# JJanai/slowflow

Hardware: AMD Instinct MI355X
Metric: Mpix*solver-iters/s at 1024x436 (whole coarse-to-fine path) (higher is better)
Workload: dtype f32

## Files before the change

slowflow_amd/csrc/api.hip:

```cpp
#include <algorithm>
#include <cmath>
#include <cstring>
#include <memory>
#include <mutex>

#include "sfa_internal.h"

#pragma clang fp contract(off)

namespace sfa {

thread_local std::string g_thread_err;

#ifndef SFA_RELEASE
Switches g_switches;
static const char *const kSwitchNames[Switches::N] = {
    "SFA_SOR_CHAIN", "SFA_SOR_BAND", "SFA_SOR_F", "SFA_SOR_CH", "SFA_SOR_LEAD", "SFA_CHAIN_LDS", "SFA_RB_TILE", "SFA_WARP_ALLJ", "SFA_NO_WARP_SMOOTH",
    "SFA_ASSEMBLE_GENERIC", "SFA_EXACT_DIV", "SFA_ASM_XCD", "SFA_NO_DIRECT_OPERANDS", "SFA_NO_UV_ALIAS", "SFA_DEBUG_ACTIVE", "SFA_UNFUSED", "SFA_SHARE_SOR",
    "SFA_PYRAMID_UNFUSED", "SFA_CUT_DISCHARGE", "SFA_CUT_INNER", "SFA_CUT_SUPER", "SFA_CUT_TAIL_INNER", "SFA_CUT_PER", "SFA_CUT_TAIL_PER", "SFA_CUT_TAIL_SUPER",
    "SFA_CUT_DEBUG", "SFA_CUT_NO_TAIL", "SFA_CUT_TAIL", "SFA_NO_EXACT_BREAK", "SFA_PAIR_UNFUSED"};
static int set_switch(const char *name, const char *value) {
    for (int i = 0; i < Switches::N; i++)
        if (!strcmp(name, kSwitchNames[i])) {
            g_switches.given[i] = value != nullptr;
            g_switches.value[i] = value ? atoi(value) : 0;
            return SFA_OK;
        }
    return SFA_ERR_ARG;
}
static void switches_from_environment() {
    static std::once_flag once;
    std::call_once(once, [] {
        const char *d = getenv("SFA_DEBUG");
        if (!d || atoi(d) == 0) return;
        for (int i = 0; i < Switches::N; i++)
            if (const char *e = getenv(kSwitchNames[i])) (void)set_switch(kSwitchNames[i], e);
    });
}
#else
static void switches_from_environment() {}
#endif

int set_error(sfa_ctx *ctx, int code, const char *fmt, ...) {
    char buf[1024];
    va_list ap;
    va_start(ap, fmt);
    vsnprintf(buf, sizeof buf, fmt, ap);
    va_end(ap);
    g_thread_err = buf;
    if (ctx) ctx->err = buf;
    return code;
}

int DevMem::alloc(sfa_ctx *ctx, size_t n) {
    if (n <= bytes && p) return SFA_OK;
    release();
    hipError_t e = hipMalloc(&p, n);
    if (e != hipSuccess) { p = nullptr; return set_error(ctx, SFA_ERR_HIP, "hipMalloc(%zu) failed: %s", n, hipGetErrorString(e)); }
    bytes = n;
    return SFA_OK;
}
void DevMem::release() {
    if (p) (void)hipFree(p);
    p = nullptr;
    bytes = 0;
}

int upload_plane(sfa_ctx *ctx, float *dev, int pitch, const float *host, int stride, int w, int h) {
    SFA_HIP(ctx, hipMemcpy2DAsync(dev, (size_t)pitch * 4, host, (size_t)stride * 4, (size_t)w * 4, h, hipMemcpyHostToDevice, ctx->stream));
    return SFA_OK;
}
int download_plane(sfa_ctx *ctx, float *host, int stride, const float *dev, int pitch, int w, int h) {
    SFA_HIP(ctx, hipMemcpy2DAsync(host, (size_t)stride * 4, dev, (size_t)pitch * 4, (size_t)w * 4, h, hipMemcpyDeviceToHost, ctx->stream));
    return SFA_OK;
}

static int check_device_error(sfa_ctx *c) {
    unsigned e = 0;
    SFA_HIP(c, hipMemcpyAsync(&e, c->d_err, sizeof e, hipMemcpyDeviceToHost, c->stream));
    SFA_HIP(c, hipStreamSynchronize(c->stream));
    if (e) {
        (void)hipMemsetAsync(c->d_err, 0, sizeof(unsigned), c->stream);
        return set_error(c, SFA_ERR_TIMEOUT, "SOR pipeline: a bounded in-kernel wait gave up (code %u)", e);
    }
    return SFA_OK;
}

int cv_gauss_taps(float sigma, float *k) {
    const int ksize = ((int)lrint((double)sigma * 4 * 2 + 1)) | 1;
    const double scale2X = -0.5 / ((double)sigma * sigma);
    double sum = 0;
    for (int i = 0; i < ksize; i++) {
        const double x = i - (ksize - 1) * 0.5;
        k[i] = (float)exp(scale2X * x * x);
        sum += k[i];
    }
    sum = 1. / sum;
    for (int i = 0; i < ksize; i++) k[i] = (float)(k[i] * sum);
    return ksize / 2;
}

}

using namespace sfa;

extern "C" {

int sfa_device_count(void) {
    int n = 0;
    if (hipGetDeviceCount(&n) != hipSuccess) return 0;
    return n;
}

int sfa_ctx_create(int device, sfa_ctx **out) {
    if (!out) return set_error(nullptr, SFA_ERR_ARG, "sfa_ctx_create: out is null");
    *out = nullptr;
    int n = 0;
    if (hipGetDeviceCount(&n) != hipSuccess || n <= 0)
        return set_error(nullptr, SFA_ERR_NO_DEVICE, "no HIP device available: slowflow_amd has no CPU fallback");
    if (device < 0 || device >= n) return set_error(nullptr, SFA_ERR_ARG, "device %d out of range (%d devices)", device, n);
    switches_from_environment();
    std::unique_ptr<sfa_ctx> c(new sfa_ctx());
    c->device = device;
    SFA_HIP(c.get(), hipSetDevice(device));
    SFA_HIP(c.get(), hipStreamCreateWithFlags(&c->stream, hipStreamNonBlocking));
    SFA_HIP(c.get(), hipMalloc((void **)&c->d_red, kRedDoubles * sizeof(double)));
    SFA_HIP(c.get(), hipHostMalloc((void **)&c->h_red, sizeof(LastBlock) + 64, hipHostMallocDefault));
    SFA_HIP(c.get(), hipMalloc((void **)&c->d_amask, 64));
    SFA_HIP(c.get(), hipMalloc((void **)&c->d_last, sizeof(LastBlock)));
    SFA_HIP(c.get(), hipMemset(c->d_last, 0, sizeof(LastBlock)));
    SFA_HIP(c.get(), hipHostMalloc((void **)&c->h_amask, kMaskRing * sizeof(WMask), hipHostMallocDefault));
    for (auto &e : c->ev_mask) SFA_HIP(c.get(), hipEventCreateWithFlags(&e, hipEventDisableTiming));
    SFA_HIP(c.get(), hipMalloc((void **)&c->d_err, 64));
    SFA_HIP(c.get(), hipMemset(c->d_err, 0, 64));
    SFA_HIP(c.get(), hipEventCreate(&c->t0));
    SFA_HIP(c.get(), hipEventCreate(&c->t1));
    SFA_HIP(c.get(), hipEventCreateWithFlags(&c->ev_wait, hipEventDisableTiming));
    SFA_HIP(c.get(), hipEventCreateWithFlags(&c->ev_signal, hipEventDisableTiming));
    hipDeviceProp_t prop;
    if (hipGetDeviceProperties(&prop, device) == hipSuccess) c->cu_count = prop.multiProcessorCount;
    *out = c.release();
    return SFA_OK;
}

void sfa_ctx_destroy(sfa_ctx *c) {
    if (!c) return;
    (void)hipSetDevice(c->device);
    (void)hipStreamSynchronize(c->stream);
    for (auto e : c->ev) (void)hipEventDestroy(e);
    for (auto e : c->ev2) (void)hipEventDestroy(e);
    if (c->t0) (void)hipEventDestroy(c->t0);
    if (c->t1) (void)hipEventDestroy(c->t1);
    if (c->ev_wait) (void)hipEventDestroy(c->ev_wait);
    if (c->ev_signal) (void)hipEventDestroy(c->ev_signal);
    if (c->d_red) (void)hipFree(c->d_red);
    if (c->h_red) (void)hipHostFree(c->h_red);
    if (c->d_err) (void)hipFree(c->d_err);
    if (c->d_amask) (void)hipFree(c->d_amask);
    if (c->d_last) (void)hipFree(c->d_last);
    if (c->h_amask) (void)hipHostFree(c->h_amask);
    for (auto e : c->ev_mask) if (e) (void)hipEventDestroy(e);
    if (c->rb_tmp) (void)hipFree(c->rb_tmp);
    if (c->q_tmp) (void)hipFree(c->q_tmp);
    if (c->stream) (void)hipStreamDestroy(c->stream);
    delete c;
}

const char *sfa_last_error(const sfa_ctx *c) { return c ? c->err.c_str() : g_thread_err.c_str(); }

int sfa_ctx_sync(sfa_ctx *c) {
    if (!c) return set_error(nullptr, SFA_ERR_ARG, "null context");
    SFA_HIP(c, hipSetDevice(c->device));
    return check_device_error(c);
// ... 774 lines not shown
```

slowflow_amd/csrc/job.hip:

```cpp
#include <algorithm>
#include <cmath>
#include <cstring>
#include <memory>
#include <vector>

#include "sfa_internal.h"

#pragma clang fp contract(off)

namespace sfa {

enum { P_WX = 0, P_WY, P_UU, P_VV, P_DU, P_DV, P_ODU, P_ODV, P_SH, P_SV, P_A11, P_A12, P_A22, P_B1, P_B2, P_OCC, P_DPSIS, P_COUNT };
struct Level {
    int w = 0, h = 0, pitch = 0, lstride = 0, ref = 0, F = 0, nb = 0;
    bool fused = true;
    long pl = 0, es = 0;
    long off_masks = 0, off_warp = 0, off_stacks = 0, off_tmp = 0;
    float *base = nullptr;
    float *pbase = nullptr;
    float *plane(int i) const { return i < 2 ? pbase + (long)i * pl : base + (long)(i - 2) * pl; }
    float *mask(int s) const { return base + off_masks + (long)s * pl; }
    float *stack(int s, int toref) const { return base + off_stacks + ((long)s * 2 + toref) * 24 * pl; }
    float *warp(int s, int sp1) const { return base + off_warp + (long)(s + sp1) * 3 * pl; }
    float *frame(int f) const { return pbase + 2 * pl + (long)f * 3 * pl; }
    float *tmp() const { return base + off_tmp; }
    Geo geo() const { return Geo{w, h, pitch, pl, es, nb, WMask::first(nb), nullptr}; }
    Geo geo(const WMask &active) const { return Geo{w, h, pitch, pl, es, nb, active, nullptr}; }
    static long persistent_floats(int pitch, int h, int ref) { return (long)pitch * h * (2 + (2L * ref + 1) * 3); }
    static long transient_floats(int pitch, int h, int ref, bool fused) {
        return (long)pitch * h * ((P_COUNT - 2) + 2 * ref + (2L * ref + 1) * 3 + (fused ? 0 : 2L * ref * 2 * 24));
    }
    void layout(float *transient, float *persistent, int w_, int h_, int lstride_, int ref_, int nb_, long es_, bool fused_) {
        base = transient; pbase = persistent; w = w_; h = h_; pitch = dev_pitch(w_); lstride = lstride_; ref = ref_; F = 2 * ref_ + 1; nb = nb_; es = es_; fused = fused_;
        pl = (long)pitch * h;
        off_masks = (long)(P_COUNT - 2) * pl;
        off_warp = off_masks + 2L * ref * pl;
        off_stacks = off_warp + (2L * ref + 1) * 3 * pl;
        off_tmp = off_warp;
    }
};
struct ChannelWeights { const float *dev = nullptr; long pl = 0, es = 0; int pitch = 0, stride0 = 0; };

static const float *pair_image(const Level &L, int s, int sp1) { return (s + sp1 - L.ref == 0) ? L.frame(s + sp1) : L.warp(s, sp1); }

static bool get_derivatives(sfa_ctx *c, const Level &L, const sfa_params &p, const Geo &g, const bool need_toref[2 * SFA_MAX_REF], bool with_smoothness = false) {
    const int ref = L.ref;
    WarpJobs J;
    J.n = 0;
    for (int f = p.one_direction ? ref + 1 : 0; f <= 2 * ref; f++) {
        if (f == ref) continue;
        const int s = f < ref ? f : f - 1;
        J.job[J.n++] = WarpJob{L.frame(f) - L.base, L.warp(f < ref ? f : f - 1, f < ref ? 0 : 1) - L.base, L.mask(s) - L.base, f - ref};
    }
    const bool smoothed = with_smoothness && L.fused &&
                          launch_warp_smooth(c, g, J, L.base, L.plane(P_WX), L.plane(P_WY), p.smoothing, L.plane(P_SH), L.plane(P_SV), L.plane(P_DPSIS), p.alpha, pen(p.robust_reg));
    if (!smoothed) launch_warp_jobs(c, g, J, L.base, L.plane(P_WX), L.plane(P_WY));
    for (int s = p.one_direction ? ref : 0; s < 2 * ref; s++) {
        if (L.fused) continue;
        const float *w_s = pair_image(L, s, 0), *w_sp1 = pair_image(L, s, 1);
        launch_deriv_stack(c, g, L.stack(s, 0), w_s, w_sp1, L.es, L.es);
        if (need_toref[s]) {
            if (s < ref) launch_deriv_stack(c, g, L.stack(s, 1), w_s, L.frame(ref), L.es, L.es);
            else         launch_deriv_stack(c, g, L.stack(s, 1), L.frame(ref), w_sp1, L.es, L.es);
        }
    }
    return smoothed;
}

static int optimize_occlusions(sfa_ctx *c, const Level &L, const sfa_params &p, const Geo &g, DevMem &scratch) {
    const int ref = L.ref;
    const size_t n = (size_t)L.nb * L.pl;
    SFA_TRY(scratch.alloc(c, (2 + kCutWorkPlanes) * n * sizeof(float)));
    float *d0 = scratch.f(), *d1 = d0 + n, *work = d1 + n;
    OccArgs oa;
    memset(&oa, 0, sizeof oa);
    oa.nslots = 2 * ref; oa.hd = p.delta / 3.0f; oa.hg = p.gamma / 3.0f; oa.penalty = p.occlusion_penalty;
    oa.color = pen(p.robust_color); oa.grad = pen(p.robust_grad);
    for (int s = 0; s < 2 * ref; s++) {
        const float *i1 = pair_image(L, s, 0), *i2 = pair_image(L, s, 1);
        const float *r1 = s < ref ? i1 : L.frame(ref), *r2 = s < ref ? L.frame(ref) : i2;
        const int idx = std::max(ref - s - 1, s - ref);
        oa.slot[s] = OccSlot{i1 - L.base, i2 - L.base, r1 - L.base, r2 - L.base, L.off_masks + (long)s * L.pl, p.rho[idx], p.omega[idx], s >= ref ? 0 : 1};
    }
    launch_occ_costs(c, g, oa, L.base, d0, d1, L.pl);
    return run_grid_cut(c, g, L.plane(P_OCC), L.es, d0, d1, work, p.occlusion_alpha);
}


static Term data_term(const Level &L, const sfa_params &p, int slot, int is_ref, float weight, float s) {
    const float *i1 = pair_image(L, slot, 0), *i2 = pair_image(L, slot, 1);
    if (is_ref) { if (slot < L.ref) i2 = L.frame(L.ref); else i1 = L.frame(L.ref); }
    return Term{L.off_stacks + ((long)slot * 2 + is_ref) * 24 * L.pl, L.off_masks + (long)slot * L.pl, weight * (p.delta / 3.0f), weight * (p.gamma / 3.0f), s, is_ref,
                i1 - L.base, i2 - L.base, slot < L.ref};
}
static int data_terms(sfa_ctx *c, const Level &L, const sfa_params &p, const ChannelWeights &cw, AssembleArgs &aa, bool need_toref[2 * SFA_MAX_REF]) {
    const int ref = L.ref;
    memset(&aa, 0, sizeof aa);
    for (int s = 0; s < ref; s++) {
        const int a = ref - 1 - s;
        if (!p.one_direction) {
            if (p.rho[a] > 0) aa.t[aa.n++] = data_term(L, p, s, 0, p.rho[a], (float)(s - ref));
            if (p.omega[a] > 0) { aa.t[aa.n++] = data_term(L, p, s, 1, p.omega[a], (float)(s - ref)); need_toref[s] = true; }
        }
        if (p.rho[s] > 0) aa.t[aa.n++] = data_term(L, p, ref + s, 0, p.rho[s], (float)s);
        if (p.omega[s] > 0) { aa.t[aa.n++] = data_term(L, p, ref + s, 1, p.omega[s], (float)(s + 1)); need_toref[ref + s] = true; }
        aa.data_norm += p.rho[s] + p.omega[s];
    }
    for (int t = 0; t < aa.n; t++)
        if (aa.t[t].is_ref && aa.t[t].s == 0) return set_error(c, SFA_ERR_REF_FRAME, "Frame compared to reference frame is the reference frame itself!");
    aa.one_direction = p.one_direction; aa.dt_norm = p.dataterm_norm;
    aa.color = pen(p.robust_color); aa.grad = pen(p.robust_grad);
    aa.chw = cw.dev; aa.chw_pl = cw.pl; aa.chw_es = cw.es; aa.chw_pitch = cw.pitch; aa.chw_stride0 = cw.stride0; aa.lstride = L.lstride;
    aa.accumulate = 0; aa.do_laplacian = 1;
    return SFA_OK;
}

struct LevelPlan {
    bool verbose;
    bool red_black;
    bool direct;
    bool uv_alias;
    bool thres_in, thres_out;
    float *wx, *wy, *uu, *vv, *du, *dv, *odu, *odv, *sh, *sv, *a11, *a12, *a22, *b1, *b2, *occ, *dpsis, *UU, *VV;
    float *dfa, *dfb, *ifa, *ifb;
    LevelPlan(const sfa_ctx *c, const Level &L, const sfa_params &p) {
        verbose = c->verbose_changes;
        red_black = p.sor_order == 1;
        direct = L.fused && !red_black && !sw_given(Switches::NO_DIRECT_OPERANDS);
        uv_alias = direct && p.niter_inner == 1 && !sw_given(Switches::NO_UV_ALIAS) && !verbose;
        thres_in = p.thres_inner > 0; thres_out = p.thres_outer > 0;
        wx = L.plane(P_WX); wy = L.plane(P_WY); uu = L.plane(P_UU); vv = L.plane(P_VV); du = L.plane(P_DU); dv = L.plane(P_DV);
        odu = L.plane(P_ODU); odv = L.plane(P_ODV); sh = L.plane(P_SH); sv = L.plane(P_SV); a11 = L.plane(P_A11); a12 = L.plane(P_A12);
        a22 = L.plane(P_A22); b1 = L.plane(P_B1); b2 = L.plane(P_B2); occ = L.plane(P_OCC); dpsis = L.plane(P_DPSIS);
        UU = uv_alias ? wx : uu; VV = uv_alias ? wy : vv;
        dfa = thres_out && !sw_given(Switches::NO_EXACT_BREAK) ? a11 : nullptr; dfb = dfa ? a12 : nullptr;
        ifa = thres_in && !sw_given(Switches::NO_EXACT_BREAK) ? a11 : nullptr; ifb = ifa ? a12 : nullptr;
    }
};

struct OuterBreak {
    sfa_ctx *c; bool on;
    int known(int n, WMask &active) const {
        if (!on || n < kMaskLag) return SFA_OK;
        const int slot = (n - kMaskLag) % kMaskRing;
        SFA_HIP(c, hipEventSynchronize(c->ev_mask[slot]));
        for (int i = 0; i < kMaskWords; i++) active.w[i] = *(volatile unsigned long long *)&c->h_amask[slot].w[i];
        return SFA_OK;
    }
    int publish(int n) const {
        if (!on) return SFA_OK;
        const int slot = n % kMaskRing;
        SFA_HIP(c, hipMemcpyAsync(&c->h_amask[slot], c->d_amask, sizeof(WMask), hipMemcpyDeviceToHost, c->stream));
        SFA_HIP(c, hipEventRecord(c->ev_mask[slot], c->stream));
        return SFA_OK;
    }
};

static void print_changes(sfa_ctx *c, const Level &L, const char *what, int it, const WMask &who) {
    if (hipMemcpyAsync(c->h_red, c->d_red, 2 * L.nb * sizeof(double), hipMemcpyDeviceToHost, c->stream) != hipSuccess || hipStreamSynchronize(c->stream) != hipSuccess) return;
    const double n = (double)L.w * L.h;
    for (int b = 0; b < L.nb; b++)
        if (who.test(b)) {
            if (L.nb > 1) printf("[window %d] ", b);
            printf("%s %d\tavg change %g,%g\n", what, it, (double)(float)(c->h_red[2 * b] / n), (double)(float)(c->h_red[2 * b + 1] / n));
        }
    fflush(stdout);
}

static int assemble_and_solve(sfa_ctx *c, const Level &L, const sfa_params &p, const LevelPlan &P, AssembleArgs &aa, SorWorkspace &sorws, const Geo &gi, bool first_zero,
                       bool smoothed) {
    if (!first_zero) launch_copy_planes(c, gi, P.odu, P.du, 2, L.es, L.es);
    if (!smoothed) launch_smoothness(c, gi, p.smoothing, P.sh, P.sv, P.UU, P.VV, P.dpsis, p.alpha, pen(p.robust_reg));
    aa.op = SorOperandOut();
    aa.zero_duv = first_zero ? 1 : 0;
    if (P.direct) SFA_TRY(sor_operand_target(c, sorws, gi, p.niter_solver, &aa.op));
    if (L.fused) SFA_TRY(launch_assemble_images(c, gi, aa, L.base, P.a11, P.a12, P.a22, P.b1, P.b2, P.du, P.dv, P.UU, P.VV, P.sh, P.sv, P.occ));
    else launch_assemble(c, gi, aa, L.base, P.a11, P.a12, P.a22, P.b1, P.b2, P.du, P.dv, P.uu, P.vv, P.sh, P.sv);
    if (P.direct) return sor_run_prepared(c, sorws, gi, nullptr, nullptr, p.niter_solver, p.sor_omega);
    if (P.red_black) return sor_rb_run(c, gi, P.du, P.dv, P.a11, P.a12, P.a22, P.b1, P.b2, P.sh, P.sv, p.niter_solver, p.sor_omega);
    return sor_run(c, sorws, gi, P.du, P.dv, P.a11, P.a12, P.a22, P.b1, P.b2, P.sh, P.sv, p.niter_solver, p.sor_omega, false);
}

static bool update_flow(sfa_ctx *c, const sfa_params &p, const LevelPlan &P, const SorOperandOut &x, const Geo &gi, int inner, bool first_zero) {
    const bool last = inner + 1 == p.niter_inner;
    float *const ia = last ? nullptr : P.ifa, *const ib = last ? nullptr : P.ifb;
    if (P.direct && last && !P.verbose) {
        launch_update_outer_x(c, gi, P.uv_alias ? nullptr : P.uu, P.uv_alias ? nullptr : P.vv, P.wx, P.wy, x, c->d_red, P.dfa, P.dfb);
        return true;
    }
    if (P.direct)
        launch_update_inner_x(c, gi, P.uu, P.vv, P.wx, P.wy, x, first_zero ? nullptr : P.odu, first_zero ? nullptr : P.odv, last ? nullptr : P.du,
                              last ? nullptr : P.dv, c->d_red, ia, ib);
    else
        launch_update_inner(c, gi, P.uu, P.vv, P.wx, P.wy, P.du, P.dv, P.odu, P.odv, c->d_red, ia, ib);
    return false;
}

static int inner_break(sfa_ctx *c, const Level &L, const sfa_params &p, const LevelPlan &P, const Geo &gi, WMask &in_active) {
    const double npx = (double)L.h * L.w;
    SFA_HIP(c, hipMemcpyAsync(c->h_red, c->d_red, 2 * L.nb * sizeof(double), hipMemcpyDeviceToHost, c->stream));
    SFA_HIP(c, hipStreamSynchronize(c->stream));
    WMask close = WMask::none();
    for (int b = 0; b < L.nb; b++)
        if (in_active.test(b)) {
            const double ad = c->h_red[2 * b] / npx, dd = c->h_red[2 * b + 1] / npx, dm = (ad < dd) ? dd : ad;
            if (P.ifa && fabs(dm - (double)p.thres_inner) <= break_band(L.w, L.h) * (double)p.thres_inner) { close.set(b); continue; }
            if (std::max((float)ad, (float)dd) < p.thres_inner) in_active.clear(b);
        }
    if (!close.any()) return SFA_OK;
    float *const dx = c->d_last->exact;
    const float *const hx = reinterpret_cast<const LastBlock *>(c->h_red)->exact;
    launch_exact_norms(c, gi, P.ifa, P.ifb, close, dx);
    SFA_HIP(c, hipMemcpyAsync(const_cast<float *>(hx), dx, 2 * L.nb * sizeof(float), hipMemcpyDeviceToHost, c->stream));
    SFA_HIP(c, hipStreamSynchronize(c->stream));
    for (int b = 0; b < L.nb; b++)
        if (close.test(b) && std::max(hx[2 * b], hx[2 * b + 1]) < p.thres_inner) in_active.clear(b);
    return SFA_OK;
}

static int inner_iterations(sfa_ctx *c, const Level &L, const sfa_params &p, const LevelPlan &P, AssembleArgs &aa, SorWorkspace &sorws, const Geo &g, bool smoothed) {
    if (!P.direct) launch_zero_planes(c, g, P.du, 2);
    WMask in_active = g.active, outer_done = WMask::none();
    for (int inner = 0; inner < p.niter_inner; inner++) {
        Geo gi = g;
        gi.active = in_active;
        const bool first_zero = P.direct && inner == 0;
        SFA_TRY(assemble_and_solve(c, L, p, P, aa, sorws, gi, first_zero, smoothed && inner == 0));
        if (update_flow(c, p, P, aa.op, gi, inner, first_zero)) outer_done = in_active;
        if (P.verbose) print_changes(c, L, "\tinner it", inner, in_active);
        if (P.thres_in && inner + 1 < p.niter_inner) {
            SFA_TRY(inner_break(c, L, p, P, gi, in_active));
            if (!in_active.any()) break;
        }
    }
    if (outer_done != g.active) {
        Geo go = g;
        go.active = g.active.andnot(outer_done);
        launch_update_outer(c, go, P.wx, P.wy, P.uu, P.vv, c->d_red, P.dfa, P.dfb);
    }
    return SFA_OK;
}
static int run_level(sfa_ctx *c, const Level &L, const sfa_params &p, const ChannelWeights &cw, SorWorkspace &sorws, DevMem &cut_scratch, float *change, float *occ_log) {
    AssembleArgs aa;
    bool need_toref[2 * SFA_MAX_REF] = {false};
    SFA_TRY(data_terms(c, L, p, cw, aa, need_toref));
    const LevelPlan P(c, L, p);
    const OuterBreak brk{c, P.thres_out};
    const WMask all = WMask::first(L.nb);
    Geo g = L.geo(all);
    launch_fill_planes(c, g, P.occ, 1, (p.one_direction || p.occlusion_reasoning) ? -1.0f : 0.0f);
    launch_dpsis(c, g, P.dpsis, L.frame(L.ref), L.es, 5.0f, p.norm_avg, p.norm_std, p.hbit);
    if (!P.uv_alias) launch_copy_planes(c, g, P.uu, P.wx, 2, L.es, L.es);
    g.amask = c->d_amask;
    SFA_HIP(c, hipMemsetAsync(c->d_last, 0, sizeof(LastBlock), c->stream));
    launch_set_mask(c, all);

    for (int alter = 0; alter < p.niter_alter; alter++) {
        WMask active = all;
        g.active = active;
        if (P.thres_out && alter > 0) launch_set_mask(c, all);
        bool smoothed = get_derivatives(c, L, p, g, need_toref, P.uv_alias);
        if (alter > 0 && p.occlusion_reasoning && !p.one_direction) SFA_TRY(optimize_occlusions(c, L, p, g, cut_scratch));
        if (alter > 0 && p.occlusion_reasoning && occ_log)
            launch_copy_planes(c, g, occ_log + (long)alter * L.pl, P.occ, 1, (long)p.niter_alter * L.pl, L.es);
        for (int outer = 0; outer < p.niter_outer; outer++) {
            SFA_TRY(brk.known(outer, active));
            if (!active.any()) break;
            if (sw_given(Switches::DEBUG_ACTIVE)) fprintf(stderr, "level %dx%d alter %d outer %d known active %d\n", L.w, L.h, alter, outer, active.count());
            g.active = active;
            if (outer > 0) smoothed = get_derivatives(c, L, p, g, need_toref, P.uv_alias);
            if (!L.fused) launch_mask_weight(c, g, L.mask(0), P.occ, aa.data_norm, L.ref, p.one_direction);
            SFA_TRY(inner_iterations(c, L, p, P, aa, sorws, g, smoothed));
            if (P.verbose) print_changes(c, L, "outer it", outer, active);
            const bool last_iter = (alter == p.niter_alter - 1 && outer == p.niter_outer - 1);
            if (P.thres_out || last_iter) launch_outer_threshold(c, g, c->d_red, P.thres_out ? p.thres_outer : 0.0f, P.dfa, P.dfb);
            SFA_TRY(brk.publish(outer));
        }
    }
    if (change) {
        SFA_HIP(c, hipMemcpyAsync(c->h_red, c->d_last->last, 2 * L.nb * sizeof(double), hipMemcpyDeviceToHost, c->stream));
        SFA_HIP(c, hipStreamSynchronize(c->stream));
        for (int i = 0; i < 2 * L.nb; i++) change[i] = (float)c->h_red[i];
    }
    return SFA_OK;
}

static int gaussian_filter_order(float sigma) {
    int order = (int)floor(3 * sigma) + 1;
    if (order == 0) order = 1;
    return order;
}
static int pyramid_sizes(int w, int h, int layers, float p_scale, int *ws, int *hs) {
    const float sigma = 1 / sqrtf(2 * p_scale);
    const int order = gaussian_filter_order(sigma);
    for (int l = 0; l < layers; l++) {
        ws[l] = l == 0 ? w : (int)(float)floor(ws[l - 1] * p_scale);
        hs[l] = l == 0 ? h : (int)(float)floor(hs[l - 1] * p_scale);
        if (floor(ws[l] * p_scale) <= order + 1 || floor(hs[l] * p_scale) <= order + 1) return l;
    }
    return layers;
}

}
using namespace sfa;

struct sfa_job {
    sfa_ctx *ctx = nullptr;
    sfa_params p;
    int w = 0, h = 0, nb = 0, ref = 0, F = 0, L = 0;
    int ws[64], hs[64];
    long es = 0;
    std::vector<long> level_off;
    long trans_off = 0;
    bool share_sor = false;
    DevMem arena;
    DevMem init_flow;
    DevMem chw;
    DevMem cut_scratch;
    bool has_chw = false;
    int chw_stride0 = 0;
    std::vector<std::unique_ptr<SorWorkspace>> sor;
    std::vector<float> change;
    double mpix_iters = 0;
    int host_stride0 = 0;
    bool fused = true;
    Level level(int l) const {
        Level Lv;
        Lv.layout(arena.f() + trans_off, arena.f() + level_off[l], ws[l], hs[l], l == 0 ? host_stride0 : host_stride(ws[l]), ref, nb, es, fused);
        return Lv;
    }
    WMask presmoothed = WMask::none();
    bool keep_alt_occ = false;
    DevMem occ_log;
    float *chw_stage = nullptr;
    hipEvent_t ev_chw = nullptr;
};

static int job_windows(sfa_ctx *ctx, const char *fn, const sfa_job *j, int b0, int n) { return check_batch_range(ctx, fn, "windows", b0, n, j->nb); }

static int job_weight_planes(sfa_job *j, int stride) {
    if (j->has_chw) return SFA_OK;
    const size_t n = (size_t)j->nb * 3 * dev_pitch(stride) * j->h;
    SFA_TRY(j->chw.alloc(j->ctx, n * sizeof(float)));
    launch_fill(j->ctx, j->chw.f(), n, 1.0f);
    j->has_chw = true;
    j->chw_stride0 = stride;
    return SFA_OK;
}
static int job_set_channel_weights(sfa_job *j, int b, int stride, const float *const chw[3]) {
    sfa_ctx *ctx = j->ctx;
    if (chw) {
        CHECK_ARGS((long)stride * j->h < (1L << 31), "channel weights: the linear pixel index must fit 31 bits");
        SFA_TRY(job_weight_planes(j, stride));
        CHECK_ARGS(j->chw_stride0 == stride, "channel weights of all elements must share one stride");
        const int cp = dev_pitch(stride);
        for (int k = 0; k < 3; k++) {
            CHECK_ARGS(chw[k], "null weight plane");
            SFA_TRY(upload_plane(ctx, j->chw.f() + ((long)b * 3 + k) * cp * j->h, cp, chw[k], stride, stride, j->h));
        }
    } else if (j->has_chw) {
        launch_fill(ctx, j->chw.f() + (long)b * 3 * dev_pitch(j->chw_stride0) * j->h, (size_t)3 * dev_pitch(j->chw_stride0) * j->h, 1.0f);
    }
    return SFA_OK;
}
static int job_upload_flow_and_weights(sfa_job *j, int b, const float *wx, const float *wy, int stride, const float *const chw[3]) {
    sfa_ctx *ctx = j->ctx;
    const Level L0 = j->level(0);
    const float *const host[2] = {wx, wy};
    for (int k = 0; k < 2; k++) {
        float *dst = j->init_flow.f() + ((long)b * 2 + k) * L0.pl;
        if (host[k]) SFA_TRY(upload_plane(ctx, dst, L0.pitch, host[k], stride, j->w, j->h));
        else SFA_HIP(ctx, hipMemsetAsync(dst, 0, L0.pl * sizeof(float), ctx->stream));
    }
    return job_set_channel_weights(j, b, stride, chw);
}
static void job_presmooth(sfa_job *j) {
    const WMask all = WMask::first(j->nb);
    if (!(j->p.presmooth_sigma > 0) || (j->presmoothed & all) == all) return;
    const Level L0 = j->level(0);
    float *tmp = L0.tmp();
    for (int f = 0; f < j->F; f++) {
        launch_presmooth(j->ctx, L0.geo(all), tmp + 3 * L0.pl, tmp, L0.frame(f), 3, j->p.presmooth_sigma);
        launch_copy_planes(j->ctx, L0.geo(all.andnot(j->presmoothed)), L0.frame(f), tmp + 3 * L0.pl, 3, L0.es, L0.es);
    }
    j->presmoothed = all;
}
static void job_pyramid(sfa_job *j) {
    sfa_ctx *ctx = j->ctx;
    const int nb = j->nb, F = j->F;
    float taps[64];
    const int radius = cv_gauss_taps(1 / sqrtf(2 * j->p.p_scale), taps);
    for (int l = 1; l < j->L; l++) {
        const Level Lp = j->level(l - 1), Lc = j->level(l);
        float *tmp = Lp.tmp();
        if (!sw_given(Switches::PYRAMID_UNFUSED) &&
            launch_pyr_down(ctx, Lc.frame(0), Lc.w, Lc.h, Lc.pitch, Lc.pl, Lc.es, Lp.frame(0), Lp.w, Lp.h, Lp.pitch, Lp.pl, Lp.es, 3 * F, nb, taps, radius))
            continue;
        for (int f = 0; f < F; f++) {
            launch_gauss_blur(ctx, Lp.geo(), tmp + 3 * Lp.pl, tmp, Lp.frame(f), 3, taps, radius);
            launch_resize(ctx, Lc.frame(f), Lc.w, Lc.h, Lc.pitch, Lc.pl, Lc.es, tmp + 3 * Lp.pl, Lp.w, Lp.h, Lp.pitch, Lp.pl, Lp.es, 3, nb, 1.0f);
        }
    }
}
static void job_initial_flow(sfa_job *j) {
    const Level L0 = j->level(0), Lt = j->level(j->L - 1);
    if (j->L > 1) {
        const float fx = (1.0f * Lt.w) / j->w, fy = (1.0f * Lt.h) / j->h;
        launch_resize_flow(j->ctx, Lt.plane(P_WX), Lt.plane(P_WY), Lt.w, Lt.h, Lt.pitch, Lt.es, j->init_flow.f(), j->init_flow.f() + L0.pl, j->w, j->h, L0.pitch, 2 * L0.pl, j->nb, fx, fy);
    } else {
        launch_copy_planes(j->ctx, L0.geo(), L0.plane(P_WX), j->init_flow.f(), 2, L0.es, 2 * L0.pl);
    }
}

extern "C" {

int sfa_pyramid_sizes(int w, int h, int layers, float p_scale, int *ws, int *hs) {
    if (layers < 1 || layers > 64 || !ws || !hs) return 0;
    return pyramid_sizes(w, h, layers, p_scale, ws, hs);
}

int sfa_job_create(sfa_ctx *ctx, const sfa_params *p, int w, int h, int batch, sfa_job **out) {
    CHECK_ARGS(ctx && p && out && w >= 2 && h >= 5 && batch > 0 && batch <= kMaxBatch, "bad arguments (h >= 5, w >= 2)");
    CHECK_ARGS(p->S >= 2 && p->S - 1 <= SFA_MAX_REF && p->layers >= 1 && p->layers <= 64, "unsupported slow_flow_S / slow_flow_layers");
    CHECK_ARGS(2L * kMaxBatch + 2L * batch * ((w + 63) / 64) * 16 <= kRedDoubles, "batch x width beyond the change norms' scratch (sfa_internal.h: kRedDoubles)");
    SFA_HIP(ctx, hipSetDevice(ctx->device));
    std::unique_ptr<sfa_job> j(new sfa_job());
    j->ctx = ctx; j->p = *p; j->w = w; j->h = h; j->nb = batch; j->ref = p->S - 1; j->F = 2 * j->ref + 1;
    j->L = pyramid_sizes(w, h, p->layers, p->p_scale, j->ws, j->hs);
    CHECK_ARGS(j->L >= 1, "image too small for even one pyramid level");
    j->fused = sw_int(Switches::UNFUSED, 0) == 0;
    long off = 0;
    double px = 0;
    for (int l = 0; l < j->L; l++) {
        j->level_off.push_back(off);
        off += Level::persistent_floats(dev_pitch(j->ws[l]), j->hs[l], j->ref);
        j->sor.emplace_back(new SorWorkspace());
        px += (double)j->ws[l] * j->hs[l];
    }
    j->trans_off = off;
    off += Level::transient_floats(dev_pitch(j->ws[0]), j->hs[0], j->ref, j->fused);
    j->es = off;
    j->share_sor = (double)w * h >= 2.0e6 || sw_given(Switches::SHARE_SOR);
    j->host_stride0 = host_stride(w);
    SFA_TRY(j->arena.alloc(ctx, (size_t)batch * j->es * sizeof(float)));
    SFA_HIP(ctx, hipMemsetAsync(j->arena.p, 0, (size_t)batch * j->es * sizeof(float), ctx->stream));
    SFA_TRY(j->init_flow.alloc(ctx, (size_t)batch * 2 * dev_pitch(w) * h * sizeof(float)));
    SFA_HIP(ctx, hipMemsetAsync(j->init_flow.p, 0, (size_t)batch * 2 * dev_pitch(w) * h * sizeof(float), ctx->stream));
    j->change.assign(2 * batch, 0.f);
    j->mpix_iters = px * p->niter_alter * p->niter_outer * p->niter_inner * p->niter_solver * batch / 1e6;
    *out = j.release();
    return SFA_OK;
}
void sfa_job_destroy(sfa_job *j) {
    if (!j) return;
    (void)hipSetDevice(j->ctx->device);
    (void)hipStreamSynchronize(j->ctx->stream);
    if (j->ev_chw) (void)hipEventDestroy(j->ev_chw);
    if (j->chw_stage) (void)hipHostFree(j->chw_stage);
    delete j;
}
double sfa_job_mpix_iters(const sfa_job *j) { return j ? j->mpix_iters : 0; }
double sfa_job_device_bytes(const sfa_job *j) {
    if (!j) return 0;
    double b = (double)j->arena.bytes + j->init_flow.bytes + j->chw.bytes + j->cut_scratch.bytes + j->occ_log.bytes;
    for (const auto &w : j->sor) b += (double)w->sa.bytes + w->sb.bytes + w->x.bytes + w->flags.bytes + w->order.bytes + w->edge.bytes;
    return b;
}

int sfa_job_upload(sfa_job *j, int b, const float *const *frames, int n_frames, const float *wx, const float *wy, int stride, const float *const chw[3]) {
    sfa_ctx *ctx = j ? j->ctx : nullptr;
    CHECK_ARGS(j && b >= 0 && b < j->nb && frames && n_frames == j->F && stride >= j->w, "bad arguments (n_frames must be 2*(S-1)+1)");
    SFA_HIP(ctx, hipSetDevice(ctx->device));
    Level L0 = j->level(0);
    j->host_stride0 = stride;
    j->presmoothed.clear(b);
    for (int f = 0; f < j->F; f++) {
        CHECK_ARGS(frames[f], "null frame");
        for (int k = 0; k < 3; k++)
            SFA_TRY(upload_plane(ctx, L0.frame(f) + b * j->es + k * L0.pl, L0.pitch, frames[f] + (size_t)k * stride * j->h, stride, j->w, j->h));
    }
    SFA_TRY(job_upload_flow_and_weights(j, b, wx, wy, stride, chw));
    SFA_HIP(ctx, hipStreamSynchronize(ctx->stream));
    return SFA_OK;
}

int sfa_job_upload_resident(sfa_job *j, int b, const sfa_sequence *q, const int *frame_index, int n_frames, const float *wx, const float *wy, int stride,
                            const float *const chw[3]) {
    sfa_ctx *ctx = j ? j->ctx : nullptr;
    CHECK_ARGS(j && q && frame_index && b >= 0 && b < j->nb && n_frames == j->F && stride >= j->w, "bad arguments (n_frames must be 2*(S-1)+1)");
    CHECK_ARGS(q->w == j->w && q->h == j->h && q->ctx->device == ctx->device, "the sequence must have the job's frame size and live on the job's GPU");
    SFA_HIP(ctx, hipSetDevice(ctx->device));
    Level L0 = j->level(0);
    j->host_stride0 = stride;
    j->presmoothed.clear(b);
    for (int f = 0; f < j->F; f++) {
        CHECK_ARGS(frame_index[f] >= 0 && frame_index[f] < q->n, "frame index out of range");
        SFA_HIP(ctx, hipMemcpyAsync(L0.frame(f) + b * j->es, q->frame(frame_index[f]), (size_t)3 * L0.pl * sizeof(float), hipMemcpyDeviceToDevice, ctx->stream));
    }
    SFA_TRY(job_upload_flow_and_weights(j, b, wx, wy, stride, chw));
    if (wx || wy || chw) SFA_HIP(ctx, hipStreamSynchronize(ctx->stream));
    return SFA_OK;
}

int sfa_job_reset_flow(sfa_job *j) { return j ? SFA_OK : SFA_ERR_ARG; }

int sfa_job_run(sfa_job *j) {
    sfa_ctx *ctx = j ? j->ctx : nullptr;
    CHECK_ARGS(j, "null job");
    SFA_HIP(ctx, hipSetDevice(ctx->device));
    job_presmooth(j);
    job_pyramid(j);
    job_initial_flow(j);
    ChannelWeights cw;
    if (j->has_chw) {
        cw.dev = j->chw.f(); cw.pitch = dev_pitch(j->chw_stride0); cw.pl = (long)cw.pitch * j->h; cw.es = 3 * cw.pl; cw.stride0 = j->chw_stride0;
    }
    for (int l = j->L - 1; l >= 0; l--) {
        Level Lc = j->level(l);
        if (l < j->L - 1) {
            Level Ln = j->level(l + 1);
            const float fx = (1.0f * Lc.w) / Ln.w, fy = (1.0f * Lc.h) / Ln.h;
            launch_resize_flow(ctx, Lc.plane(P_WX), Lc.plane(P_WY), Lc.w, Lc.h, Lc.pitch, Lc.es, Ln.plane(P_WX), Ln.plane(P_WY), Ln.w, Ln.h, Ln.pitch, Ln.es, j->nb, fx, fy);
        }
        SFA_TRY(run_level(ctx, Lc, j->p, cw, *j->sor[j->share_sor ? 0 : l], j->cut_scratch, l == 0 ? j->change.data() : nullptr, l == 0 && j->keep_alt_occ ? j->occ_log.f() : nullptr));
    }
    SFA_HIP(ctx, hipGetLastError());
    return SFA_OK;
}

int sfa_job_download(sfa_job *j, int b, float *wx, float *wy, int stride, float change[2]) {
    sfa_ctx *ctx = j ? j->ctx : nullptr;
    CHECK_ARGS(j && b >= 0 && b < j->nb && wx && wy && stride >= j->w, "bad arguments");
    SFA_HIP(ctx, hipSetDevice(ctx->device));
    Level L0 = j->level(0);
    SFA_TRY(download_plane(ctx, wx, stride, L0.plane(P_WX) + b * j->es, L0.pitch, j->w, j->h));
    SFA_TRY(download_plane(ctx, wy, stride, L0.plane(P_WY) + b * j->es, L0.pitch, j->w, j->h));
    if (change) { change[0] = j->change[2 * b]; change[1] = j->change[2 * b + 1]; }
    return sfa_ctx_sync(ctx);
}

int sfa_job_keep_alternation_occlusions(sfa_job *j, int on) {
    sfa_ctx *ctx = j ? j->ctx : nullptr;
    CHECK_ARGS(j, "null job");
    SFA_HIP(ctx, hipSetDevice(ctx->device));
    j->keep_alt_occ = on != 0;
    if (on) {
        const size_t n = (size_t)j->nb * std::max(1, j->p.niter_alter) * dev_pitch(j->w) * j->h * sizeof(float);
        SFA_TRY(j->occ_log.alloc(ctx, n));
        SFA_HIP(ctx, hipMemsetAsync(j->occ_log.p, 0, n, ctx->stream));
    }
    return SFA_OK;
}

int sfa_job_download_alternation_occlusions(sfa_job *j, int b, int alter, float *occ, int stride) {
    sfa_ctx *ctx = j ? j->ctx : nullptr;
    CHECK_ARGS(j && b >= 0 && b < j->nb && occ && stride >= j->w, "bad arguments");
    CHECK_ARGS(j->keep_alt_occ && j->occ_log.p, "sfa_job_keep_alternation_occlusions was not enabled before the run");
    CHECK_ARGS(alter >= 1 && alter < j->p.niter_alter, "alternation out of range: labels exist for 1 <= alter < niter_alter (variational_mt.cpp:269)");
    SFA_HIP(ctx, hipSetDevice(ctx->device));
    const int pitch = dev_pitch(j->w);
    const long pl = (long)pitch * j->h;
    SFA_TRY(download_plane(ctx, occ, stride, j->occ_log.f() + ((long)b * j->p.niter_alter + alter) * pl, pitch, j->w, j->h));
    return sfa_ctx_sync(ctx);
}

int sfa_job_download_occlusions(sfa_job *j, int b, float *occ, int stride) {
    sfa_ctx *ctx = j ? j->ctx : nullptr;
    CHECK_ARGS(j && b >= 0 && b < j->nb && occ && stride >= j->w, "bad arguments");
    SFA_HIP(ctx, hipSetDevice(ctx->device));
    Level L0 = j->level(0);
    SFA_TRY(download_plane(ctx, occ, stride, L0.plane(P_OCC) + b * j->es, L0.pitch, j->w, j->h));
    return sfa_ctx_sync(ctx);
}

int sfa_job_upload_device(sfa_job *j, int b0, int n, const void *frames_dev, const sfa_dev_layout *l, const float *const chw[3]) {
    sfa_ctx *ctx = j ? j->ctx : nullptr;
    CHECK_ARGS(j, "job is null");
    SFA_HIP(ctx, hipSetDevice(ctx->device));
    SFA_TRY(job_windows(ctx, __func__, j, b0, n));
    SFA_TRY(check_frames_source(ctx, __func__, frames_dev, l, l ? l->window : 0, n, j->F, j->w, j->h));
    const int stride = host_stride(j->w);
    if (chw) {
        CHECK_ARGS(chw[0] && chw[1] && chw[2], "chw holds a null weight plane");
        CHECK_ARGS(!j->has_chw || j->chw_stride0 == stride, "chw: the job already holds channel weights of another stride");
    }
    Level L0 = j->level(0);
    j->host_stride0 = stride;
    for (int b = b0; b < b0 + n; b++) j->presmoothed.clear(b);
    const PackSrc src{frames_dev, l->dtype, l->window, l->frame, l->channel, l->row, l->column};
    launch_pack_frames(ctx, L0.frame(0) + (long)b0 * j->es, j->es, L0.pl, L0.pitch, j->w, j->h, n, j->F, src);
    if (chw) {
        const size_t plane = (size_t)stride * j->h;
        if (!j->chw_stage) {
            SFA_HIP(ctx, hipHostMalloc((void **)&j->chw_stage, 3 * plane * sizeof(float), hipHostMallocDefault));
            SFA_HIP(ctx, hipEventCreateWithFlags(&j->ev_chw, hipEventDisableTiming));
        } else {
            SFA_HIP(ctx, hipEventSynchronize(j->ev_chw));
        }
// ... 88 lines not shown
```

slowflow_amd/csrc/kernels.hip:

```cpp
#include "sfa_device.h"
#include "sor_device.h"

#pragma clang fp contract(off)

namespace sfa {

__device__ __forceinline__ float psi_vec(const PenaltyDev &p, float xsq) {
    const float e2 = p.eps * p.eps;
    switch (p.id) {
    case 0: return 1.0f;
    case 2: return __fdiv_rn(1.0f, 2.0f * e2 + xsq);
    case 3: {
        float out = __fdiv_rn(1.0f, 2.0f * sqrt_rn(xsq + e2));
        if (sqrt_rn(xsq) > p.trunc) out = 0.0f;
        return out;
    }
    case 4: {
        float t = e2 + xsq;
        t = t * t;
        return __fdiv_rn(e2 + 2.0f * xsq, t);
    }
    default: return __fdiv_rn(1.0f, 2.0f * sqrt_rn(xsq + e2));
    }
}
// ... 547 lines not shown
        tmp = uxsq + vxsq;
        outh = (float)((double)((dps(x, y) + dps(x + 1, y)) * half_alpha) / __dsqrt_rn((double)(tmp + EPS2F)));
    }
    if (y < h - 1) {
        const float uy1 = uu(x, y + 1) - uu(x, y), vy1 = vv(x, y + 1) - vv(x, y);
        float tmp = 0.5f * (d3x(uu, x, y, w) + d3x(uu, x, y + 1, w));
        const float uysq = uy1 * uy1 + tmp * tmp;
        tmp = 0.5f * (d3x(vv, x, y, w) + d3x(vv, x, y + 1, w));
        const float vysq = vy1 * vy1 + tmp * tmp;
        tmp = uysq + vysq;
        outv = (float)((double)((dps(x, y) + dps(x, y + 1)) * half_alpha) / __dsqrt_rn((double)(tmp + EPS2F)));
    }
    sh[o] = outh;
    sv[o] = outv;
}
void launch_smoothness_2f(sfa_ctx *c, const Geo &g, float *sh, float *sv, const float *uu, const float *vv, const float *dpsis, float half_alpha) {
    dim3 grid((g.pitch + BX - 1) / BX, (g.h + BY - 1) / BY, g.nb);
    hipLaunchKernelGGL(k_smoothness_2f, grid, block2d(), 0, c->stream, sh, sv, uu, vv, dpsis, g, half_alpha);
}
struct Deriv2f { float ix[3], iy[3], iz[3], ixx[3], ixy[3], iyy[3], ixz[3], iyz[3]; };
__device__ __forceinline__ void data_2f_pixel(const Deriv2f &D, float u, float v, float m, float hd, float hg, const PlaneAcc &U, const PlaneAcc &V, const PlaneAcc &H,
                                              const PlaneAcc &W, int x, int y, int w, int h, float &A11, float &A12, float &A22, float &B1, float &B2) {
    const float *ix = D.ix, *iy = D.iy, *iz = D.iz, *ixx = D.ixx, *ixy = D.ixy, *iyy = D.iyy, *ixz = D.ixz, *iyz = D.iyz;
    const float dn = 0.1f * 0.1f;
    A11 = 0.0f; A12 = 0.0f; A22 = 0.0f; B1 = 0.0f; B2 = 0.0f;
    if (hd) {
        float t[3], n[3];
#pragma unroll
        for (int k = 0; k < 3; k++) { t[k] = iz[k] + ix[k] * u + iy[k] * v; n[k] = ix[k] * ix[k] + iy[k] * iy[k] + dn; }
        const float q = __fdiv_rn(m * hd, sqrt_rn(__fdiv_rn(t[0] * t[0], n[0]) + __fdiv_rn(t[1] * t[1], n[1]) + __fdiv_rn(t[2] * t[2], n[2]) + EPS2F));
#pragma unroll
        for (int k = 0; k < 3; k++) {
            const float tk = __fdiv_rn(q, n[k]);
            A11 += tk * ix[k] * ix[k]; A12 += tk * ix[k] * iy[k]; A22 += tk * iy[k] * iy[k];
            B1 -= tk * iz[k] * ix[k];  B2 -= tk * iz[k] * iy[k];
        }
    }
    float t[6], n[6];
#pragma unroll
    for (int k = 0; k < 3; k++) {
        n[2 * k] = ixx[k] * ixx[k] + ixy[k] * ixy[k] + dn;
        n[2 * k + 1] = iyy[k] * iyy[k] + ixy[k] * ixy[k] + dn;
        t[2 * k] = ixz[k] + ixx[k] * u + ixy[k] * v;
        t[2 * k + 1] = iyz[k] + ixy[k] * u + iyy[k] * v;
    }
    const float q = __fdiv_rn(m * hg, sqrt_rn(__fdiv_rn(t[0] * t[0], n[0]) + __fdiv_rn(t[1] * t[1], n[1]) + __fdiv_rn(t[2] * t[2], n[2]) + __fdiv_rn(t[3] * t[3], n[3]) +
                                              __fdiv_rn(t[4] * t[4], n[4]) + __fdiv_rn(t[5] * t[5], n[5]) + EPS2F));
#pragma unroll
    for (int k = 0; k < 3; k++) {
        const float ta = __fdiv_rn(q, n[2 * k]), tb = __fdiv_rn(q, n[2 * k + 1]);
        A11 += ta * ixx[k] * ixx[k] + tb * ixy[k] * ixy[k];
        A12 += ta * ixx[k] * ixy[k] + tb * ixy[k] * iyy[k];
        A22 += tb * iyy[k] * iyy[k] + ta * ixy[k] * ixy[k];
        B1 -= ta * ixx[k] * ixz[k] + tb * ixy[k] * iyz[k];
        B2 -= tb * iyy[k] * iyz[k] + ta * ixy[k] * ixz[k];
    }
    B1 = laplacian_gather(B1, U, H, W, x, y, w, h);
    B2 = laplacian_gather(B2, V, H, W, x, y, w, h);
}
__global__ void __launch_bounds__(BX *BY) k_data_2f(const float *__restrict__ D, const float *__restrict__ mask, const float *__restrict__ du, const float *__restrict__ dv,
                                                     float *__restrict__ a11, float *__restrict__ a12, float *__restrict__ a22, float *__restrict__ b1, float *__restrict__ b2,
                                                     const float *__restrict__ wx, const float *__restrict__ wy, const float *__restrict__ sh, const float *__restrict__ sv,
                                                     Geo g, float hd, float hg) {
    const int b = blockIdx.z;
    const int x = blockIdx.x * BX + threadIdx.x, y = blockIdx.y * BY + threadIdx.y;
    if (x >= g.w || y >= g.h) return;
    const long eb = b * g.es;
    const size_t o = (size_t)y * g.pitch + x;
    const float *S = D + eb + o;
    Deriv2f d;
#pragma unroll
    for (int k = 0; k < 3; k++) {
        d.ix[k] = S[(0 * 3 + k) * g.pl]; d.iy[k] = S[(1 * 3 + k) * g.pl]; d.iz[k] = S[(2 * 3 + k) * g.pl];
        d.ixx[k] = S[(3 * 3 + k) * g.pl]; d.ixy[k] = S[(4 * 3 + k) * g.pl]; d.iyy[k] = S[(5 * 3 + k) * g.pl];
        d.ixz[k] = S[(6 * 3 + k) * g.pl]; d.iyz[k] = S[(7 * 3 + k) * g.pl];
    }
    const float u = du[eb + o], v = dv[eb + o], m = mask[eb + o];
    PlaneAcc U{wx + eb, g.pitch}, V{wy + eb, g.pitch}, H{sh + eb, g.pitch}, W{sv + eb, g.pitch};
    float A11, A12, A22, B1, B2;
    data_2f_pixel(d, u, v, m, hd, hg, U, V, H, W, x, y, g.w, g.h, A11, A12, A22, B1, B2);
    a11[eb + o] = A11; a12[eb + o] = A12; a22[eb + o] = A22; b1[eb + o] = B1; b2[eb + o] = B2;
}
void launch_data_2f(sfa_ctx *c, const Geo &g, const float *D, const float *mask, const float *du, const float *dv, float *a11, float *a12, float *a22, float *b1,
                    float *b2, const float *wx, const float *wy, const float *sh, const float *sv, float hd, float hg) {
    hipLaunchKernelGGL(k_data_2f, grid2d(g), block2d(), 0, c->stream, D, mask, du, dv, a11, a12, a22, b1, b2, wx, wy, sh, sv, g, hd, hg);
}

constexpr int DF_NT = 256, DF_ROWS = DT_Y / (DF_NT / DT_X);
__global__ void __launch_bounds__(DF_NT) k_data_2f_fused(const float *__restrict__ I1, const float *__restrict__ I2, const float *__restrict__ mask,
                                                         const float *__restrict__ du, const float *__restrict__ dv, float *__restrict__ a11, float *__restrict__ a12,
                                                         float *__restrict__ a22, float *__restrict__ b1, float *__restrict__ b2, const float *__restrict__ wx,
                                                         const float *__restrict__ wy, const float *__restrict__ sh, const float *__restrict__ sv, Geo g, float hd, float hg) {
    __shared__ float sM[DT_R * DT_W], sZ[DT_R * DT_W], sX[DT_R * DT_W], sY[DT_R * DT_W];
    const int b = blockIdx.z;
    const long eb = b * g.es;
    const int x0 = blockIdx.x * DT_X - DT_H, y0 = blockIdx.y * DT_Y - DT_H;
    const int x = x0 + DT_H + (threadIdx.x & (DT_X - 1)), yt = y0 + DT_H + threadIdx.x / DT_X;
    const bool col = x < g.w;
    Deriv2f d[DF_ROWS];
#pragma unroll
    for (int ch = 0; ch < 3; ch++) {
        const float *a = I1 + eb + ch * g.pl, *bb = I2 + eb + ch * g.pl;
        if (ch) __syncthreads();
        for (int i = threadIdx.x; i < DT_R * DT_W; i += DF_NT) {
            const int sx = x0 + i % DT_W, sy = y0 + i / DT_W;
            if (sx >= 0 && sx < g.w && sy >= 0 && sy < g.h) {
                const size_t o = (size_t)sy * g.pitch + sx;
                const float va = a[o], vb = bb[o];
                sM[i] = 0.5f * (vb + va);
                sZ[i] = va - vb;
            }
        }
        __syncthreads();
        const TileAcc m{sM, x0, y0};
        constexpr int W1 = DT_X + 4, R1 = DT_Y + 4;
        for (int i = threadIdx.x; i < R1 * W1; i += DF_NT) {
            const int lx = 2 + i % W1, ly = 2 + i / W1;
            const int sx = x0 + lx, sy = y0 + ly;
            if (sx >= 0 && sx < g.w && sy >= 0 && sy < g.h) {
                sX[ly * DT_W + lx] = d5x(m, sx, sy, g.w);
                sY[ly * DT_W + lx] = d5y(m, sx, sy, g.h);
            }
        }
        __syncthreads();
        const TileAcc ix{sX, x0, y0}, iy{sY, x0, y0}, iz{sZ, x0, y0};
#pragma unroll
        for (int r = 0; r < DF_ROWS; r++) {
            const int y = yt + r * (DF_NT / DT_X);
            if (col && y < g.h) {
                d[r].ix[ch] = ix(x, y); d[r].iy[ch] = iy(x, y); d[r].iz[ch] = iz(x, y);
                d[r].ixx[ch] = d5x(ix, x, y, g.w); d[r].ixy[ch] = d5y(ix, x, y, g.h); d[r].iyy[ch] = d5y(iy, x, y, g.h);
                d[r].ixz[ch] = d5x(iz, x, y, g.w); d[r].iyz[ch] = d5y(iz, x, y, g.h);
            }
        }
    }
    if (!col) return;
    PlaneAcc U{wx + eb, g.pitch}, V{wy + eb, g.pitch}, H{sh + eb, g.pitch}, W{sv + eb, g.pitch};
#pragma unroll
    for (int r = 0; r < DF_ROWS; r++) {
        const int y = yt + r * (DF_NT / DT_X);
        if (y >= g.h) break;
        const size_t o = (size_t)y * g.pitch + x;
        float A11, A12, A22, B1, B2;
        data_2f_pixel(d[r], du[eb + o], dv[eb + o], mask[eb + o], hd, hg, U, V, H, W, x, y, g.w, g.h, A11, A12, A22, B1, B2);
        a11[eb + o] = A11; a12[eb + o] = A12; a22[eb + o] = A22; b1[eb + o] = B1; b2[eb + o] = B2;
    }
}
void launch_data_2f_fused(sfa_ctx *c, const Geo &g, const float *I1, const float *I2, const float *mask, const float *du, const float *dv, float *a11, float *a12,
                          float *a22, float *b1, float *b2, const float *wx, const float *wy, const float *sh, const float *sv, float hd, float hg) {
    hipLaunchKernelGGL(k_data_2f_fused, dim3((g.w + DT_X - 1) / DT_X, (g.h + DT_Y - 1) / DT_Y, g.nb), dim3(DF_NT), 0, c->stream, I1, I2, mask, du, dv, a11, a12, a22, b1,
                       b2, wx, wy, sh, sv, g, hd, hg);
}

__device__ __forceinline__ void mask_weights(float oc, float data_norm, float &fwd, float &bwd) {
    float factor = (oc == 0.0f) ? 1.0f : 0.0f;
    factor = (1 + factor) * data_norm;
    bwd = __fdiv_rn((oc >= 0.0f) ? 1.0f : 0.0f, factor);
    fwd = __fdiv_rn((oc <= 0.0f) ? 1.0f : 0.0f, factor);
}
__global__ void k_mask_weight(float *__restrict__ masks, const float *__restrict__ occ, Geo g, float data_norm, int ref, int one_direction) {
    const int b = blockIdx.z;
    if (!elem_active(g, b)) return;
    const int x = blockIdx.x * BX + threadIdx.x, y = blockIdx.y * BY + threadIdx.y;
    if (x >= g.w || y >= g.h) return;
    const size_t o = (size_t)y * g.pitch + x;
    float forward, backward;
    mask_weights(occ[b * g.es + o], data_norm, forward, backward);
    for (int s = one_direction ? ref : 0; s < 2 * ref; s++) {
        float *m = masks + b * g.es + s * g.pl + o;
        *m = (s < ref) ? 1.0f * backward * (*m) : 1.0f * forward * (*m);
    }
}
void launch_mask_weight(sfa_ctx *c, const Geo &g, float *masks, const float *occ, float data_norm, int ref, int one_direction) {
    hipLaunchKernelGGL(k_mask_weight, grid2d(g), block2d(), 0, c->stream, masks, occ, g, data_norm, ref, one_direction);
}

__global__ void k_fill(float *p, size_t n, float v) {
    size_t i = (size_t)blockIdx.x * blockDim.x + threadIdx.x;
    const size_t step = (size_t)gridDim.x * blockDim.x;
    for (; i < n; i += step) p[i] = v;
}
void launch_fill(sfa_ctx *c, float *p, size_t n, float v) {
    if (!n) return;
    const int blocks = (int)std::min<size_t>((n + 255) / 256, 4096);
    hipLaunchKernelGGL(k_fill, dim3(blocks), dim3(256), 0, c->stream, p, n, v);
}

#define DATANORM (0.1f * 0.1f)


struct Recip { float b, r; };
__device__ __forceinline__ Recip recip_of(float b) {
    float r = __builtin_amdgcn_rcpf(b);
    const float e = __builtin_fmaf(-b, r, 1.0f);
    r = __builtin_fmaf(e, r, r);
    return Recip{b, r};
}
__device__ __forceinline__ float div_by(float a, const Recip &d) {
    float q = a * d.r;
    float e = __builtin_fmaf(-d.b, q, a);
    q = __builtin_fmaf(e, d.r, q);
    e = __builtin_fmaf(-d.b, q, a);
    return __builtin_fmaf(e, d.r, q);
}
__device__ __forceinline__ bool wave_all(bool ok) { return __builtin_amdgcn_ballot_w64(!ok) == 0ull; }
__device__ __forceinline__ unsigned num_key(float a) { return __float_as_uint(a) - 1u; }
constexpr unsigned kNumLo = 0x14000000u - 1u;
constexpr float kNumHi = 9007199254740992.0f, kDenHi = 8589934592.0f;
__device__ __forceinline__ bool num_ok(float a) { return (int)__float_as_uint(a) >= 0 && num_key(a) >= kNumLo && a < kNumHi; }
__device__ __forceinline__ bool num_ok3(float a, float b, float c) {
    const unsigned ka = num_key(a), kb = num_key(b), kc = num_key(c);
    return min(ka, min(kb, kc)) >= kNumLo && fmaxf(a, fmaxf(b, c)) < kNumHi;
}
__device__ __forceinline__ bool den_ok3(float a, float b, float c) { return fmaxf(a, fmaxf(b, c)) < kDenHi; }
#ifdef SFA_EXACT_DIV_ONLY
#define SFA_FAST_DIV(cond) false
#else
#define SFA_FAST_DIV(cond) (SHDIV && chain && wave_all(cond))
#endif

__global__ void k_division_chain(const float *__restrict__ a, const float *__restrict__ b, float *__restrict__ q_chain, float *__restrict__ q_exact,
                                 unsigned char *__restrict__ admitted, size_t n) {
    for (size_t i = (size_t)blockIdx.x * blockDim.x + threadIdx.x; i < n; i += (size_t)gridDim.x * blockDim.x) {
        const float x = a[i], y = b[i];
        q_chain[i] = div_by(x, recip_of(y));
        q_exact[i] = __fdiv_rn(x, y);
        admitted[i] = (num_ok(x) && den_ok3(y, y, y) && y >= 7.450580596923828125e-9f) ? 1 : 0;
    }
}
void launch_division_chain(sfa_ctx *c, const float *a, const float *b, float *q_chain, float *q_exact, unsigned char *admitted, size_t n) {
    hipLaunchKernelGGL(k_division_chain, dim3(2048), dim3(256), 0, c->stream, a, b, q_chain, q_exact, admitted, n);
}

struct Acc { float a11, a12, a22, b1, b2; };

struct Px {
    float wk[3], ix[3], iy[3], iz[3], ixx[3], ixy[3], iyy[3], ixz[3], iyz[3];
};

template <bool ZUV = false, bool SHDIV = false>
__device__ __forceinline__ void term_succ(Acc &A, const Px &p, float m, float u, float v, float hd, float hg, float s, int dt_norm,
                                          const PenaltyDev &color, const PenaltyDev &grad, bool chain = false) {
    const float factor = s, factorp1 = s + 1;
    if (hd) {
        float r[3], tx[3], ty[3];
#pragma unroll
        for (int k = 0; k < 3; k++) {
            r[k] = ZUV ? p.wk[k] * p.iz[k]
                       : p.wk[k] * (p.iz[k] + p.ix[k] * factor * u + p.iy[k] * factor * v - p.ix[k] * factorp1 * u - p.iy[k] * factorp1 * v);
            tx[k] = factor * p.ix[k] - factorp1 * p.ix[k];
            ty[k] = factor * p.iy[k] - factorp1 * p.iy[k];
        }
        if (!dt_norm) {
            const float t = m * hd * psi_vec(color, r[0] * r[0] + r[1] * r[1] + r[2] * r[2]);
#pragma unroll
            for (int k = 0; k < 3; k++) {
                const float t2 = t * p.wk[k];
                A.a11 += t2 * tx[k] * tx[k];
                A.a12 += t2 * tx[k] * ty[k];
                A.a22 += t2 * ty[k] * ty[k];
                A.b1 -= t2 * p.iz[k] * tx[k];
                A.b2 -= t2 * p.iz[k] * ty[k];
            }
        } else {
            float n[3];
#pragma unroll
            for (int k = 0; k < 3; k++) n[k] = tx[k] * tx[k] + ty[k] * ty[k] + DATANORM;
            const float a0 = r[0] * r[0], a1 = r[1] * r[1], a2 = r[2] * r[2];
            const bool f1 = SFA_FAST_DIV(num_ok3(a0, a1, a2) && den_ok3(n[0], n[1], n[2]));
            Recip d[3];
            float q0, q1, q2;
            if (f1) {
#pragma unroll
                for (int k = 0; k < 3; k++) d[k] = recip_of(n[k]);
                q0 = div_by(a0, d[0]); q1 = div_by(a1, d[1]); q2 = div_by(a2, d[2]);
            } else { q0 = __fdiv_rn(a0, n[0]); q1 = __fdiv_rn(a1, n[1]); q2 = __fdiv_rn(a2, n[2]); }
            const float t = m * hd * psi_vec(color, q0 + q1 + q2);
            const bool f2 = f1;
#pragma unroll
            for (int k = 0; k < 3; k++) {
                float tk = f2 ? div_by(t, d[k]) : __fdiv_rn(t, n[k]);
                tk = tk * p.wk[k];
                A.a11 += tk * tx[k] * tx[k];
                A.a12 += tk * tx[k] * ty[k];
                A.a22 += tk * ty[k] * ty[k];
                A.b1 -= tk * p.iz[k] * tx[k];
                A.b2 -= tk * p.iz[k] * ty[k];
            }
        }
    }
    float r[6], X[3], Y[3], Z[3];
#pragma unroll
    for (int k = 0; k < 3; k++) {
        r[2 * k] = ZUV ? p.wk[k] * p.ixz[k]
                       : p.wk[k] * (p.ixz[k] + p.ixx[k] * factor * u + p.ixy[k] * factor * v - p.ixx[k] * factorp1 * u - p.ixy[k] * factorp1 * v);
        r[2 * k + 1] = ZUV ? p.wk[k] * p.iyz[k]
                           : p.wk[k] * (p.iyz[k] + p.ixy[k] * factor * u + p.iyy[k] * factor * v - p.ixy[k] * factorp1 * u - p.iyy[k] * factorp1 * v);
        X[k] = factor * p.ixx[k] - factorp1 * p.ixx[k];
        Y[k] = factor * p.iyy[k] - factorp1 * p.iyy[k];
        Z[k] = factor * p.ixy[k] - factorp1 * p.ixy[k];
    }
    if (!dt_norm) {
        const float t = m * hg * psi_vec(grad, r[0] * r[0] + r[1] * r[1] + r[2] * r[2] + r[3] * r[3] + r[4] * r[4] + r[5] * r[5]);
#pragma unroll
        for (int k = 0; k < 3; k++) {
            const float t2 = t * p.wk[k];
            A.a11 += t2 * X[k] * X[k] + t2 * Z[k] * Z[k];
            A.a12 += t2 * X[k] * Z[k] + t2 * Z[k] * Y[k];
            A.a22 += t2 * Y[k] * Y[k] + t2 * Z[k] * Z[k];
            A.b1 -= t2 * p.ixz[k] * X[k] + t2 * p.iyz[k] * Z[k];
            A.b2 -= t2 * p.iyz[k] * Y[k] + t2 * p.ixz[k] * Z[k];
        }
// ... 297 lines not shown
    float *const lds = asm_lds<K>();
    for (int part = ty; part < K::NSI; part += K::NR) {
        const int k = part * 64 + tx;
        const int q = k % K::QM, ly = (k / K::QM) % K::TR, ch = k / (K::QM * K::TR);
        const int gy = y0 + ly, gx = x0 + 4 * q;
        if (!(SFA_X_AI & 1) && k < K::NSQ && gy >= 0 && gy < g.h && gx >= 0 && gx + 3 < g.w) {
            const unsigned po = 4u * ((unsigned)ch * (unsigned)g.pl + (unsigned)gy * (unsigned)g.pitch + (unsigned)gx);
            const unsigned ld = lds_addr(lds + 256 * part);
            dma16s(I1, po, ld);
            dma16s(I2, po, ld + 4u * K::ZOFF);
        }
    }
}
template <class K, bool INTERIOR>
__device__ __forceinline__ void asm_convert(const float *I1, const float *I2, const Geo &g, int x0, int y0) {
    float *const lds = asm_lds<K>();
    for (int item = threadIdx.x; item < ((SFA_X_AI & 2) ? 0 : K::NSQ); item += K::NT) {
        float4 *const m = reinterpret_cast<float4 *>(lds + 4 * item), *const z = reinterpret_cast<float4 *>(lds + K::ZOFF + 4 * item);
        int gx = 0;
        size_t row = 0;
        bool staged = true, iz = true;
        if (!INTERIOR) {
            const int q = item % K::QM, ly = (item / K::QM) % K::TR, ch = item / (K::QM * K::TR);
            const int gy = y0 + ly;
            if (gy < 0 || gy >= g.h) continue;
            gx = x0 + 4 * q;
            row = ch * g.pl + (size_t)gy * g.pitch;
            staged = gx >= 0 && gx + 3 < g.w;
            iz = ly >= 2 && ly < K::TR - 2;
        }
        float4 va, vb;
        if (staged) { va = *m; vb = *z; }
        else {
            auto clamped = [&](const float *r) { return make_float4(r[clampi(gx, 0, g.w - 1)], r[clampi(gx + 1, 0, g.w - 1)], r[clampi(gx + 2, 0, g.w - 1)], r[clampi(gx + 3, 0, g.w - 1)]); };
            va = clamped(I1 + row); vb = clamped(I2 + row);
        }
        *m = make_float4(0.5f * (vb.x + va.x), 0.5f * (vb.y + va.y), 0.5f * (vb.z + va.z), 0.5f * (vb.w + va.w));
        if (iz) *z = make_float4(va.x - vb.x, va.y - vb.y, va.z - vb.z, va.w - vb.w);
    }
}
struct QuadXY { float X[4], Y[4]; };
__device__ __forceinline__ QuadXY quad_taps(const float *Mq, bool x_in, bool y_in) {
    QuadXY d = {};
    const float2 lo = *reinterpret_cast<const float2 *>(Mq - 2), hi = *reinterpret_cast<const float2 *>(Mq + 4);
    const float4 mid = *reinterpret_cast<const float4 *>(Mq);
    const float m2[8] = {lo.x, lo.y, mid.x, mid.y, mid.z, mid.w, hi.x, hi.y};
    if (x_in) {
#pragma unroll
        for (int e = 0; e < 4; e++) d.X[e] = tap5(m2[e], m2[e + 1], m2[e + 2], m2[e + 3], m2[e + 4]);
    }
    if (y_in) {
        const float4 r0 = *reinterpret_cast<const float4 *>(Mq - 2 * DT_W), r1 = *reinterpret_cast<const float4 *>(Mq - DT_W);
        const float4 r3 = *reinterpret_cast<const float4 *>(Mq + DT_W), r4 = *reinterpret_cast<const float4 *>(Mq + 2 * DT_W);
        d.Y[0] = tap5(r0.x, r1.x, m2[2], r3.x, r4.x); d.Y[1] = tap5(r0.y, r1.y, m2[3], r3.y, r4.y);
        d.Y[2] = tap5(r0.z, r1.z, m2[4], r3.z, r4.z); d.Y[3] = tap5(r0.w, r1.w, m2[5], r3.w, r4.w);
    }
    return d;
}
template <class K, bool INTERIOR>
__device__ __forceinline__ void asm_stage1(const Geo &g, int x0, int y0) {
    float *const lds = asm_lds<K>();
    float *const sX = lds + K::XOFF, *const sY = sX + 3 * K::N1;
    for (int item = threadIdx.x; item < ((SFA_X_AI & 4) ? 0 : K::AT_R1 * 3 * K::Q1); item += K::NT) {
        QuadXY d;
        int out = 4 * item;
        if (INTERIOR) {
            const int ch = (item >= K::AT_R1 * K::Q1 ? 1 : 0) + (item >= 2 * K::AT_R1 * K::Q1 ? 1 : 0);
            d = quad_taps(lds + 4 * item + 2 * DT_W + (K::NM - K::N1) * ch, true, true);
        } else {
            const int q = item % K::Q1, ch = (item / K::Q1) % 3, ly = item / (3 * K::Q1);
            const int gy = y0 + 2 + ly, gx = x0 + 4 * q;
            if (gy < 0 || gy >= g.h) continue;
            const float *M = lds + ch * K::NM;
            const int c = (ly + 2) * DT_W + 4 * q;
            const bool x_in = gx >= 0 && gx + 3 < g.w, y_in = gy >= 2 && gy + 2 < g.h;
            d = quad_taps(M + c, x_in, y_in);
            if (!x_in) {
#pragma unroll
                for (int e = 0; e < 4; e++) d.X[e] = d5x_in(M, c + e + (clampi(gx + e, 0, g.w - 1) - (gx + e)));
            }
            if (!y_in) {
                const TileAcc m4{M, x0, y0};
#pragma unroll
                for (int e = 0; e < 4; e++) d.Y[e] = d5y(m4, clampi(gx + e, 0, g.w - 1), gy, g.h);
            }
            out = ch * K::N1 + ly * DT_W + 4 * q;
        }
        *reinterpret_cast<float4 *>(sX + out) = make_float4(d.X[0], d.X[1], d.X[2], d.X[3]);
        *reinterpret_cast<float4 *>(sY + out) = make_float4(d.Y[0], d.Y[1], d.Y[2], d.Y[3]);
    }
}
template <class K>
__device__ __forceinline__ Px asm_pixel_derivatives(const Geo &g, int x0, int y0, int tx, int yl, int y) {
    Px p;
    const float *const lds = asm_lds<K>();
    const float(*sZ)[K::NM] = reinterpret_cast<const float(*)[K::NM]>(lds + K::ZOFF);
    const float(*sX)[K::N1] = reinterpret_cast<const float(*)[K::N1]>(lds + K::XOFF), (*sY)[K::N1] = sX + 3;
    int txl = tx;
    asm volatile("" : "+v"(txl));
    const int c = (yl + 2) * DT_W + (txl + 4);
    const int cz = (yl + 4) * DT_W + (txl + 4);
    int cb = K::ZOFF + c;
    asm volatile("" : "+v"(cb));
    const float *const pX = lds + cb + (K::XOFF - K::ZOFF), *const pY = pX + 3 * K::N1, *const pZ = lds + cb + 2 * DT_W;
    if (SFA_X_AI & 8) {
#pragma unroll
        for (int ch = 0; ch < 3; ch++) {
            p.ixy[ch] = sX[ch][c + 1]; p.iyy[ch] = sY[ch][c + 1]; p.iyz[ch] = sZ[ch][cz + 1];
            p.ix[ch] = sX[ch][c]; p.iy[ch] = sY[ch][c]; p.iz[ch] = sZ[ch][cz]; p.ixx[ch] = sX[ch][c - 1]; p.ixz[ch] = sZ[ch][cz - 1];
        }
    } else if (y >= 2 && y + 2 < g.h) {
        float xr[3][5], xc[3][4], yc[3][5], zr[3][5], zc[3][4];
        auto read_taps = [&](int ch) {
            const float *X = pX + ch * K::N1, *Y = pY + ch * K::N1, *Z = pZ + ch * K::NM;
#pragma unroll
            for (int j = 0; j < 5; j++) xr[ch][j] = X[j - 2];
            xc[ch][0] = X[-2 * DT_W]; xc[ch][1] = X[-DT_W]; xc[ch][2] = X[DT_W]; xc[ch][3] = X[2 * DT_W];
#pragma unroll
            for (int j = 0; j < 5; j++) yc[ch][j] = Y[(j - 2) * DT_W];
#pragma unroll
            for (int j = 0; j < 5; j++) zr[ch][j] = Z[j - 2];
            zc[ch][0] = Z[-2 * DT_W]; zc[ch][1] = Z[-DT_W]; zc[ch][2] = Z[DT_W]; zc[ch][3] = Z[2 * DT_W];
        };
        auto filters = [&](int ch) {
            p.ix[ch] = xr[ch][2]; p.iy[ch] = yc[ch][2]; p.iz[ch] = zr[ch][2];
            p.ixx[ch] = tap5(xr[ch][0], xr[ch][1], xr[ch][2], xr[ch][3], xr[ch][4]);
            p.ixy[ch] = tap5(xc[ch][0], xc[ch][1], xr[ch][2], xc[ch][2], xc[ch][3]);
            p.iyy[ch] = tap5(yc[ch][0], yc[ch][1], yc[ch][2], yc[ch][3], yc[ch][4]);
            p.ixz[ch] = tap5(zr[ch][0], zr[ch][1], zr[ch][2], zr[ch][3], zr[ch][4]);
            p.iyz[ch] = tap5(zc[ch][0], zc[ch][1], zr[ch][2], zc[ch][2], zc[ch][3]);
        };
        read_taps(0); read_taps(1);
        __builtin_amdgcn_sched_barrier(0);
        filters(0);
        __builtin_amdgcn_sched_barrier(0);
        read_taps(2);
        __builtin_amdgcn_sched_barrier(0);
        filters(1); filters(2);
    } else {
        const int xl = x0 + DT_H + txl, xc_ = xl < g.w ? xl : g.w - 1;
#pragma unroll
        for (int ch = 0; ch < 3; ch++) {
            const TileAcc X{sX[ch], x0, y0 + 2}, Y{sY[ch], x0, y0 + 2}, Z{sZ[ch], x0, y0};
            p.ixy[ch] = d5y(X, xc_, y, g.h);
            p.iyy[ch] = d5y(Y, xc_, y, g.h);
            p.iyz[ch] = d5y(Z, xc_, y, g.h);
            p.ix[ch] = sX[ch][c]; p.iy[ch] = sY[ch][c]; p.iz[ch] = sZ[ch][cz];
            p.ixx[ch] = d5x_in(sX[ch], c);
            p.ixz[ch] = d5x_in(sZ[ch], cz);
        }
    }
    return p;
}
template <class K>
__device__ __forceinline__ void asm_epilogue_pixel(const AssembleArgs &a, const Geo &g, Acc &A, float u, float v, int x0, int y0, int tx, int yl, int x, int y) {
    const float *const lds = asm_lds<K>();
    const int gy0 = y0 + DT_H - 1;
    const TileAcc U{lds, x0, gy0}, V{lds + K::GR * DT_W, x0, gy0}, Hh{lds + 2 * K::GR * DT_W, x0, gy0}, Wv{lds + 3 * K::GR * DT_W, x0, gy0};
    if (a.do_laplacian) {
        A.b1 = laplacian_gather(A.b1, U, Hh, Wv, x, y, g.w, g.h);
        A.b2 = laplacian_gather(A.b2, V, Hh, Wv, x, y, g.w, g.h);
    }
    if (!a.op.sa) return;
    const float hp = Hh(x, y);
    const float hl = x > 0 ? Hh(x - 1, y) : 0.0f;
    const float vp = Wv(x, y);
    const float vt = y > 0 ? Wv(x, y - 1) : 0.0f;
    const PointBlock q = sor_point_block(hl, hp, vt, vp, y, g.h, A.a11, A.a12, A.a22);
    const OperandTile<K> T;
    T.A[yl][tx] = make_float4(q.i11, q.i12, q.i22, vt);
    T.B[yl][tx] = make_float4(A.b1, A.b2, hp, y < g.h - 1 ? vp : 0.0f);
    T.X[yl][tx] = make_float2(u, v);
}
template <class K>
__device__ __forceinline__ void asm_store_operand_tile(const SorOperandOut &op, const Geo &g, int b, int c0, int r0) {
    const OperandTile<K> T;
    for (int item = threadIdx.x; item < (DT_X + K::TY - 1) * K::TY; item += K::NT) {
        const int dl = item / K::TY, rl = item % K::TY, cl = dl - rl;
        if (cl < 0 || cl >= DT_X) continue;
        const int r = r0 + rl, c = c0 + cl;
        if (r >= g.h || c >= g.w) continue;
        const size_t e = diag_entry(b, op.ent, op.RP, op.G, c, r);
        if (SFA_X_AI & 64) continue;
        const float2 xv = T.X[rl][cl];
        op.sa[e] = T.A[rl][cl];
        op.sb[e] = T.B[rl][cl];
        op.x[e] = f2u(xv.x, xv.y);
    }
}

template <int TY, int NT, int MINB, bool ZUV, int FAST, bool XT>
__global__ void __launch_bounds__(NT, MINB) k_assemble_images(AssembleArgs a, const float *__restrict__ base, float *__restrict__ a11, float *__restrict__ a12,
                                                              float *__restrict__ a22, float *__restrict__ b1, float *__restrict__ b2,
                                                              const float *__restrict__ du, const float *__restrict__ dv, const float *__restrict__ uu,
                                                              const float *__restrict__ vv, const float *__restrict__ sh, const float *__restrict__ sv,
                                                              const float *__restrict__ occ, Geo g, XcdTiles xt) {
    using K = AsmTile<TY, NT>;
    constexpr int NR = K::NR, NP = K::NP;
    float *const lds = asm_lds<K>();
#ifdef SFA_ASM_TIMING
    unsigned long long at_acc[14] = {0}, at_t = __builtin_readcyclecounter();
#endif
    int bx, by, b;
    if (!asm_block_tile<XT>(g, xt, bx, by, b)) return;
    asm_reset_progress<K>(a.op, bx, by, b);
    if (!elem_active(g, b)) return;
    const int x0 = bx * DT_X - DT_H, y0 = by * TY - DT_H;
    const bool tile_in = SFA_TILE_FAST && x0 >= 0 && x0 + DT_W <= g.w && y0 >= 0 && y0 + K::TR <= g.h;
    const long eb = b * g.es;
    const int tx = threadIdx.x & 63;
    const int ty = __builtin_amdgcn_readfirstlane(threadIdx.x >> 6);
    const int x = x0 + DT_H + tx;
    const int dt_norm = FAST ? 1 : a.dt_norm;
    PenaltyDev pcolor = a.color, pgrad = a.grad;
    if (FAST) { pcolor.id = FAST; pgrad.id = FAST; }
    Acc A[NP];
    float u[NP], v[NP], wk[NP][3], fwd[NP], bwd[NP], oc[NP];
    bool ok[NP];
#pragma unroll
    for (int k = 0; k < NP; k++) {
        const int y = y0 + DT_H + ty + NR * k;
        ok[k] = x < g.w && y < g.h;
        A[k].a11 = A[k].a12 = A[k].a22 = A[k].b1 = A[k].b2 = 0.0f;
        u[k] = v[k] = 0.0f; fwd[k] = bwd[k] = 0.0f; oc[k] = 0.0f;
        wk[k][0] = wk[k][1] = wk[k][2] = 1.0f;
        if (!ok[k]) continue;
        const size_t o = (size_t)y * g.pitch + x;
        if (!ZUV) { u[k] = du[eb + o]; v[k] = dv[eb + o]; }
        if (!FAST && a.chw) channel_weights(a, b, x, y, wk[k]);
        if (!(SFA_X_AI & 128)) oc[k] = occ[eb + o];
    }
    const bool need_g = a.do_laplacian || a.op.sa;
    auto stage_epilogue_operands = [&]() {
        if (!need_g) return;
        for (int i0 = 0; i0 < K::NGQ; i0 += NT) {
            const int item = i0 + (int)threadIdx.x;
            const int q = item % K::QM, row = (item / K::QM) % K::GR, pl = item / (K::QM * K::GR);
            const int gy = y0 + DT_H - 1 + row, gx = x0 + 4 * q;
            const float *src = pl == 0 ? uu : pl == 1 ? vv : pl == 2 ? sh : sv;
            if (!(SFA_X_AI & 32) && item < K::NGQ && gy >= 0 && gy < g.h && gx >= 0 && gx + 3 < g.pitch && (pl >= 2 || a.do_laplacian))
                dma16(src + eb + (size_t)gy * g.pitch + gx, lds_addr(lds + 4 * (i0 + 64 * ty)));
        }
    };
    AT_MARK(13);
    if (a.n == 0) stage_epilogue_operands();
    float mk[NP];
    for (int t = 0; t < a.n; t++) {
        const Term &T = a.t[t];
        AT_MARK(0);
        if (t > 0) __syncthreads();
        AT_MARK(1);
        SFA_PRIO(SFA_PRIO_STAGE);
        asm_issue_image_dma<K>(base + eb + T.i1_off, base + eb + T.i2_off, g, x0, y0, tx, ty);
#pragma unroll
        for (int k = 0; k < NP; k++) {
            const size_t o = (size_t)(y0 + DT_H + ty + NR * k) * g.pitch + x;
            mk[k] = ok[k] && !(SFA_X_AI & 128) ? base[eb + T.mask_off + o] : 0.0f;
        }
        AT_MARK(2);
        asm volatile("s_waitcnt vmcnt(0)" ::: "memory");
#pragma unroll
        for (int k = 0; k < NP; k++) {
            asm volatile("" : "+v"(mk[k]), "+v"(oc[k]));
            if (!FAST) asm volatile("" : "+v"(wk[k][0]), "+v"(wk[k][1]), "+v"(wk[k][2]));
            if (!ZUV) asm volatile("" : "+v"(u[k]), "+v"(v[k]));
        }
        AT_MARK(3);
        __syncthreads();
        AT_MARK(4);
        if (t == 0) {
#pragma unroll
            for (int k = 0; k < NP; k++) mask_weights(oc[k], a.data_norm, fwd[k], bwd[k]);
        }
        if (tile_in) asm_convert<K, true>(base + eb + T.i1_off, base + eb + T.i2_off, g, x0, y0);
        else asm_convert<K, false>(base + eb + T.i1_off, base + eb + T.i2_off, g, x0, y0);
        AT_MARK(5);
        AT_MARK(0);
        __syncthreads();
        AT_MARK(6);
        SFA_PRIO(SFA_PRIO_STAGE);
        if (tile_in) asm_stage1<K, true>(g, x0, y0);
        else asm_stage1<K, false>(g, x0, y0);
        AT_MARK(7);
        __syncthreads();
        AT_MARK(8);
        SFA_PRIO(0);
        if (t == a.n - 1) stage_epilogue_operands();
#pragma unroll
        for (int k = 0; k < NP; k++) {
            const int yl = ty + NR * k, y = y0 + DT_H + yl;
            if (y >= g.h) break;
            Px p = asm_pixel_derivatives<K>(g, x0, y0, tx, yl, y);
#pragma unroll
            for (int ch = 0; ch < 3; ch++) p.wk[ch] = FAST ? 1.0f : wk[k][ch];
            if (!ok[k]) continue;
            float m = mk[k];
            if (!a.one_direction || !T.backward) m = T.backward ? 1.0f * bwd[k] * m : 1.0f * fwd[k] * m;
            if (SFA_X_AI & 16) {
                for (int ch = 0; ch < 3; ch++) {
                    A[k].a11 += p.ix[ch] + p.ixx[ch] + m; A[k].a12 += p.iy[ch] + p.ixy[ch]; A[k].a22 += p.iz[ch] + p.iyy[ch]; A[k].b1 += p.ixz[ch]; A[k].b2 += p.iyz[ch];
                }
            } else if (T.is_ref) term_ref<ZUV, FAST != 0>(A[k], p, m, u[k], v[k], T.hd, T.hg, T.s, dt_norm, pcolor, pgrad, a.chain_ok != 0);
            else          term_succ<ZUV, FAST != 0>(A[k], p, m, u[k], v[k], T.hd, T.hg, T.s, dt_norm, pcolor, pgrad, a.chain_ok != 0);
        }
    }
    AT_MARK(0);
    if (need_g) {
        asm volatile("s_waitcnt vmcnt(0)" ::: "memory");
        __syncthreads();
    }
    AT_MARK(9);
    SFA_PRIO(SFA_PRIO_STAGE);
#pragma unroll
    for (int k = 0; k < NP; k++) {
        if (!ok[k]) continue;
        const int yl = ty + NR * k, y = y0 + DT_H + yl;
        asm_epilogue_pixel<K>(a, g, A[k], u[k], v[k], x0, y0, tx, yl, x, y);
        if (!a.op.sa) {
            const size_t o = eb + (size_t)y * g.pitch + x;
            a11[o] = A[k].a11; a12[o] = A[k].a12; a22[o] = A[k].a22; b1[o] = A[k].b1; b2[o] = A[k].b2;
        }
    }
    if (!a.op.sa) return;
    AT_MARK(10);
    __syncthreads();
    AT_MARK(11);
    asm_store_operand_tile<K>(a.op, g, b, x0 + DT_H, y0 + DT_H);
#ifdef SFA_ASM_TIMING
    AT_MARK(12);
    if ((threadIdx.x & 63) == 0 && (bx + 3 * by + 7 * b) % 61 == 0)
        for (int i = 0; i < 14; i++) atomicAdd(&g_asm_timing[i], at_acc[i]);
#endif
}
using AsmKernel = decltype(&k_assemble_images<kAsmTY, kAsmNT, kAsmMinWaves, true, 1, true>);
template <bool ZUV, int FAST>
static AsmKernel asm_kernel(bool xcd) {
    return xcd ? k_assemble_images<kAsmTY, kAsmNT, kAsmMinWaves, ZUV, FAST, true> : k_assemble_images<kAsmTY, kAsmNT, kAsmMinWaves, ZUV, FAST, false>;
}
int launch_assemble_images(sfa_ctx *c, const Geo &g, const AssembleArgs &a_in, const float *base, float *a11, float *a12, float *a22, float *b1, float *b2,
                           const float *du, const float *dv, const float *uu, const float *vv, const float *sh, const float *sv, const float *occ) {
    AssembleArgs a = a_in;
    if ((unsigned long long)g.pl * 12ull >= (1ull << 32)) return set_error(c, SFA_ERR_ARG, "k_assemble_images: plane of %ld entries is beyond the kernel's 32-bit offsets", g.pl);
    const bool prof = c->profile && c->ev2_used + 2 <= c->ev2.size();
    if (prof) (void)hipEventRecord(c->ev2[c->ev2_used], c->stream);
    auto is_modl1 = [](int id) { return id != 0 && id != 2 && id != 3 && id != 4; };
    const bool foldable = a.dt_norm == 1 && !a.chw && !sw_given(Switches::ASSEMBLE_GENERIC);
    const int fast = !foldable ? 0 : (is_modl1(a.color.id) && is_modl1(a.grad.id)) ? 1 : (a.color.id == 2 && a.grad.id == 2) ? 2 : 0;
    {
        auto in = [](float v, float lo, float hi) { return v >= lo && v <= hi; };
        const float elo = fast == 2 ? 1.0f / 1024 : 1.0f / 1048576, ehi = fast == 2 ? 1024.0f : 1048576.0f, hlo = fast == 2 ? 1.0f / 4096 : 1.0f / 65536;
        bool okp = fast != 0 && in(a.data_norm, 1.0f / 256, 256.0f) && in(a.color.eps, elo, ehi) && in(a.grad.eps, elo, ehi);
        for (int t = 0; t < a.n && okp; t++) okp = (a.t[t].hd == 0.0f || in(a.t[t].hd, hlo, 65536.0f)) && (a.t[t].hg == 0.0f || in(a.t[t].hg, hlo, 65536.0f));
        a.chain_ok = okp && !sw_given(Switches::EXACT_DIV) ? 1 : 0;
    }
    const dim3 grid_((g.w + DT_X - 1) / DT_X, (g.h + kAsmTY - 1) / kAsmTY, g.nb);
    const bool xcd_env = sw_int(Switches::ASM_XCD, 1) != 0;
    const long ntiles = (long)grid_.x * grid_.y * grid_.z;
    const bool xcd = xcd_env && ntiles >= 64 && ntiles < (1l << 30);
    const XcdTiles xt{(int)grid_.x, (int)grid_.y, (int)((ntiles + 7) / 8)};
    const dim3 grid1_(8u * (unsigned)xt.chunk, 1, 1);
    const AsmKernel kern = a.zero_duv ? (fast == 1 ? asm_kernel<true, 1>(xcd) : fast == 2 ? asm_kernel<true, 2>(xcd) : asm_kernel<true, 0>(xcd))
                                      : (fast == 1 ? asm_kernel<false, 1>(xcd) : fast == 2 ? asm_kernel<false, 2>(xcd) : asm_kernel<false, 0>(xcd));
    hipLaunchKernelGGL(kern, xcd ? grid1_ : grid_, dim3(kAsmNT), 0, c->stream, a, base, a11, a12, a22, b1, b2, du, dv, uu, vv, sh, sv, occ, g, xt);
    if (prof) {
        (void)hipEventRecord(c->ev2[c->ev2_used + 1], c->stream);
        c->ev2_used += 2;
        c->asm_pixel_terms += (double)g.w * g.h * g.nb * a.n;
    }
    return SFA_OK;
}

__device__ __forceinline__ double wave_sum(double v) {
#pragma unroll
    for (int off = 32; off > 0; off >>= 1) v += __shfl_down(v, off, 64);
    return v;
}
__device__ __forceinline__ void block_sum2(double &a, double &b) {
    __shared__ double sm[2 * BY];
    a = wave_sum(a);
    b = wave_sum(b);
    const int wid = threadIdx.y, lane = threadIdx.x;
    if (lane == 0) { sm[wid] = a; sm[BY + wid] = b; }
    __syncthreads();
    if (wid == 0 && lane == 0) {
        double sa = 0, sb = 0;
        for (int i = 0; i < BY; i++) { sa += sm[i]; sb += sm[BY + i]; }
        a = sa; b = sb;
    }
}

__global__ void __launch_bounds__(BX *BY) k_update_inner(float *__restrict__ uu, float *__restrict__ vv, const float *__restrict__ wx, const float *__restrict__ wy,
                                                          const float *__restrict__ du, const float *__restrict__ dv, const float *__restrict__ odu,
                                                          const float *__restrict__ odv, double *__restrict__ partial, float *__restrict__ dfa, float *__restrict__ dfb, Geo g) {
    const int b = blockIdx.z;
    const int x = blockIdx.x * BX + threadIdx.x;
    double sa = 0, sb = 0;
    if (elem_active(g, b) && x < g.w)
        for (int y = blockIdx.y * BY + threadIdx.y; y < g.h; y += gridDim.y * BY) {
            const size_t o = b * g.es + (size_t)y * g.pitch + x;
            const float d = du[o], e = dv[o];
            sa += (double)fabsf(odu[o] - d);
            sb += (double)fabsf(odv[o] - e);
            if (dfa) { dfa[o] = fabsf(odu[o] - d); dfb[o] = fabsf(odv[o] - e); }
            uu[o] = wx[o] + d;
            vv[o] = wy[o] + e;
        }
    block_sum2(sa, sb);
    if (threadIdx.x == 0 && threadIdx.y == 0) {
        const size_t blk = ((size_t)b * gridDim.y + blockIdx.y) * gridDim.x + blockIdx.x;
        partial[2 * blk] = sa; partial[2 * blk + 1] = sb;
    }
}
__global__ void __launch_bounds__(BX *BY) k_update_inner_x(float *__restrict__ uu, float *__restrict__ vv, const float *__restrict__ wx, const float *__restrict__ wy,
                                                            const unsigned long long *__restrict__ xs, long ent, int RP, int G, const float *__restrict__ odu,
                                                            const float *__restrict__ odv, float *__restrict__ du_out, float *__restrict__ dv_out,
                                                            double *__restrict__ partial, float *__restrict__ dfa, float *__restrict__ dfb, Geo g) {
    const int b = blockIdx.z;
    const int x = blockIdx.x * BX + threadIdx.x;
    double sa = 0, sb = 0;
    if (elem_active(g, b) && x < g.w)
        for (int y = blockIdx.y * BY + threadIdx.y; y < g.h; y += gridDim.y * BY) {
            const size_t o = b * g.es + (size_t)y * g.pitch + x;
            const unsigned long long xv = xs[diag_entry(b, ent, RP, G, x, y)];
            const float d = __uint_as_float((unsigned)(xv & 0xffffffffu)), e = __uint_as_float((unsigned)(xv >> 32));
            const float od = odu ? odu[o] : 0.0f, oe = odv ? odv[o] : 0.0f;
            sa += (double)fabsf(od - d);
            sb += (double)fabsf(oe - e);
            if (dfa) { dfa[o] = fabsf(od - d); dfb[o] = fabsf(oe - e); }
            uu[o] = wx[o] + d;
            vv[o] = wy[o] + e;
            if (du_out) { du_out[o] = d; dv_out[o] = e; }
        }
    block_sum2(sa, sb);
    if (threadIdx.x == 0 && threadIdx.y == 0) {
        const size_t blk = ((size_t)b * gridDim.y + blockIdx.y) * gridDim.x + blockIdx.x;
        partial[2 * blk] = sa; partial[2 * blk + 1] = sb;
    }
}
template <bool FUSE>
__global__ void __launch_bounds__(BX *BY) k_update_outer_x(float *__restrict__ uu, float *__restrict__ vv, float *__restrict__ wx, float *__restrict__ wy,
                                                            const unsigned long long *__restrict__ xs, long ent, int RP, int G, double *__restrict__ partial,
                                                            double *__restrict__ out, unsigned *__restrict__ done, float *__restrict__ dfa, float *__restrict__ dfb, Geo g) {
    __shared__ unsigned long long tX[16][67];
    const int b = blockIdx.z;
    const int tid = threadIdx.y * BX + threadIdx.x;
    const int c0 = blockIdx.x * 64;
    double sa = 0, sb = 0;
    if (!elem_active(g, b)) return;
    {
        for (int r0 = blockIdx.y * 16; r0 < g.h; r0 += gridDim.y * 16) {
            __syncthreads();
            for (int item = tid; item < (64 + 16 - 1) * 16; item += BX * BY) {
                const int dl = item / 16, rl = item % 16, cl = dl - rl;
                if (cl < 0 || cl >= 64) continue;
                const int r = r0 + rl, c = c0 + cl;
                if (r < g.h && c < g.w) tX[rl][cl] = xs[diag_entry(b, ent, RP, G, c, r)];
            }
            __syncthreads();
            const int x = c0 + threadIdx.x;
            if (x < g.w)
#pragma unroll
                for (int k = 0; k < 4; k++) {
                    const int rl = threadIdx.y + 4 * k, y = r0 + rl;
                    if (y >= g.h) break;
                    const size_t o = b * g.es + (size_t)y * g.pitch + x;
                    const unsigned long long xv = tX[rl][threadIdx.x];
                    const float d = __uint_as_float((unsigned)(xv & 0xffffffffu)), e = __uint_as_float((unsigned)(xv >> 32));
                    const float ox = wx[o], oy = wy[o];
                    const float u = ox + d, v = oy + e;
                    sa += (double)fabsf(u - ox);
                    sb += (double)fabsf(v - oy);
                    if (uu) { uu[o] = u; vv[o] = v; }
                    if (dfa) { dfa[o] = fabsf(u - ox); dfb[o] = fabsf(v - oy); }
#if defined(SFA_UPD_NT) && SFA_UPD_NT
                    __builtin_nontemporal_store(u, wx + o); __builtin_nontemporal_store(v, wy + o);
#else
                    wx[o] = u; wy[o] = v;
#endif
                }
        }
    }
    block_sum2(sa, sb);
    if (!FUSE) {
        if (tid == 0) {
            const size_t blk = ((size_t)b * gridDim.y + blockIdx.y) * gridDim.x + blockIdx.x;
            partial[2 * blk] = sa; partial[2 * blk + 1] = sb;
        }
        return;
    }
    __shared__ unsigned s_last;
    const int per_elem = gridDim.x * gridDim.y;
    if (tid == 0) {
        const size_t blk = ((size_t)b * gridDim.y + blockIdx.y) * gridDim.x + blockIdx.x;
        __hip_atomic_store(&partial[2 * blk], sa, __ATOMIC_RELAXED, __HIP_MEMORY_SCOPE_AGENT);
        __hip_atomic_store(&partial[2 * blk + 1], sb, __ATOMIC_RELAXED, __HIP_MEMORY_SCOPE_AGENT);
        asm volatile("s_waitcnt vmcnt(0)" ::: "memory");
        s_last = __hip_atomic_fetch_add(&done[b], 1u, __ATOMIC_RELAXED, __HIP_MEMORY_SCOPE_AGENT) == (unsigned)(per_elem - 1);
    }
    __syncthreads();
    if (!s_last) return;
    if (tid == 0) __hip_atomic_store(&done[b], 0u, __ATOMIC_RELAXED, __HIP_MEMORY_SCOPE_AGENT);
    double ra = 0, rb = 0;
    for (int i = tid; i < per_elem; i += BX * BY) {
        ra += __hip_atomic_load(&partial[2 * ((size_t)b * per_elem + i)], __ATOMIC_RELAXED, __HIP_MEMORY_SCOPE_AGENT);
        rb += __hip_atomic_load(&partial[2 * ((size_t)b * per_elem + i) + 1], __ATOMIC_RELAXED, __HIP_MEMORY_SCOPE_AGENT);
    }
    static_assert(BX * BY == 256, "k_reduce_partials' order");
    double *s0 = reinterpret_cast<double *>(&tX[0][0]), *s1 = s0 + 256;
    __syncthreads();
    s0[tid] = ra; s1[tid] = rb;
    __syncthreads();
    for (int off = 128; off > 0; off >>= 1) {
        if (tid < off) { s0[tid] += s0[tid + off]; s1[tid] += s1[tid + off]; }
        __syncthreads();
    }
    if (tid == 0) { out[2 * b] = s0[0]; out[2 * b + 1] = s1[0]; }
}
__global__ void __launch_bounds__(BX *BY) k_update_outer(float *__restrict__ wx, float *__restrict__ wy, const float *__restrict__ uu, const float *__restrict__ vv,
                                                          double *__restrict__ partial, float *__restrict__ dfa, float *__restrict__ dfb, Geo g) {
    const int b = blockIdx.z;
    const int x = blockIdx.x * BX + threadIdx.x;
    double sa = 0, sb = 0;
    if (elem_active(g, b) && x < g.w)
        for (int y = blockIdx.y * BY + threadIdx.y; y < g.h; y += gridDim.y * BY) {
            const size_t o = b * g.es + (size_t)y * g.pitch + x;
            const float u = uu[o], v = vv[o];
            sa += (double)fabsf(u - wx[o]);
            sb += (double)fabsf(v - wy[o]);
            if (dfa) { dfa[o] = fabsf(u - wx[o]); dfb[o] = fabsf(v - wy[o]); }
            wx[o] = u;
            wy[o] = v;
        }
    block_sum2(sa, sb);
    if (threadIdx.x == 0 && threadIdx.y == 0) {
        const size_t blk = ((size_t)b * gridDim.y + blockIdx.y) * gridDim.x + blockIdx.x;
        partial[2 * blk] = sa; partial[2 * blk + 1] = sb;
    }
}
__global__ void k_reduce_partials(const double *__restrict__ partial, int per_elem, double *__restrict__ out, WMask active,
                                  const unsigned long long *__restrict__ amask) {
    const int b = blockIdx.x;
    if (!elem_active(active, amask, b)) return;
    double sa = 0, sb = 0;
    for (int i = threadIdx.x; i < per_elem; i += 256) { sa += partial[2 * ((size_t)b * per_elem + i)]; sb += partial[2 * ((size_t)b * per_elem + i) + 1]; }
    __shared__ double s0[256], s1[256];
    s0[threadIdx.x] = sa; s1[threadIdx.x] = sb;
    __syncthreads();
    for (int off = 128; off > 0; off >>= 1) {
        if (threadIdx.x < off) { s0[threadIdx.x] += s0[threadIdx.x + off]; s1[threadIdx.x] += s1[threadIdx.x + off]; }
        __syncthreads();
    }
    if (threadIdx.x == 0) { out[2 * b] = s0[0]; out[2 * b + 1] = s1[0]; }
}

__global__ void __launch_bounds__(64) k_outer_threshold(const double *__restrict__ red, double *__restrict__ last, unsigned long long *__restrict__ amask,
                                                        WMask active, int nb, double npx, float thres, unsigned long long *__restrict__ unsure, double band) {
    const int word = blockIdx.x, b = 64 * word + (int)threadIdx.x;
    const unsigned long long cur = amask[word] & active.w[word];
    bool met = false, close = false;
    if (b < nb && ((cur >> threadIdx.x) & 1ull)) {
        const double a = red[2 * b] / npx, d = red[2 * b + 1] / npx;
        last[2 * b] = a; last[2 * b + 1] = d;
        const float fa = (float)a, fd = (float)d;
        const float mx = (fa < fd) ? fd : fa;
        met = thres > 0.0f && mx < thres;
        const double dm = (a < d) ? d : a;
        close = unsure && thres > 0.0f && fabs(dm - (double)thres) <= band * (double)thres;
        if (close) met = false;
    }
    const unsigned long long m = __ballot(met), u = __ballot(close);
    if (threadIdx.x == 0) {
        amask[word] = amask[word] & ~m;
        if (unsure) unsure[word] = u;
    }
}
__device__ __forceinline__ void exact_norms(const float *__restrict__ pa, const float *__restrict__ pb, const Geo &g, int lane, float &fa, float &fd) {
    const int nblk = (g.w + 3) / 4;
    float acc_a = 0.0f, acc_b = 0.0f;
    for (int y = 0; y < g.h; y++)
        for (int b0 = 0; b0 < nblk; b0 += 64) {
            const int blk = b0 + lane, x = 4 * blk;
            float sa = 0.0f, sb = 0.0f;
            if (blk < nblk) {
                const float4 qa = *reinterpret_cast<const float4 *>(pa + (size_t)y * g.pitch + x), qb = *reinterpret_cast<const float4 *>(pb + (size_t)y * g.pitch + x);
                const float a0 = qa.x, a1 = x + 1 < g.w ? qa.y : 0.0f, a2 = x + 2 < g.w ? qa.z : 0.0f, a3 = x + 3 < g.w ? qa.w : 0.0f;
                const float c0 = qb.x, c1 = x + 1 < g.w ? qb.y : 0.0f, c2 = x + 2 < g.w ? qb.z : 0.0f, c3 = x + 3 < g.w ? qb.w : 0.0f;
                sa = ((a0 + a1) + a2) + a3;
                sb = ((c0 + c1) + c2) + c3;
            }
            const int n = min(64, nblk - b0);
            for (int i = 0; i < n; i++) {
                acc_a = acc_a + __int_as_float(__builtin_amdgcn_readlane(__float_as_int(sa), i));
                acc_b = acc_b + __int_as_float(__builtin_amdgcn_readlane(__float_as_int(sb), i));
            }
        }
    const float npx = (float)(g.h * g.w);
    fa = __fdiv_rn(acc_a, npx); fd = __fdiv_rn(acc_b, npx);
}
__global__ void __launch_bounds__(64) k_exact_break(const float *__restrict__ dfa, const float *__restrict__ dfb, double *__restrict__ last,
                                                    unsigned long long *__restrict__ amask, const unsigned long long *__restrict__ unsure, Geo g, float thres) {
    const int b = blockIdx.x, lane = threadIdx.x;
    if (!((unsure[b >> 6] >> (b & 63)) & 1ull)) return;
    float fa, fd;
    exact_norms(dfa + b * g.es, dfb + b * g.es, g, lane, fa, fd);
    if (lane == 0) {
        last[2 * b] = (double)fa; last[2 * b + 1] = (double)fd;
        const float mx = (fa < fd) ? fd : fa;
        if (mx < thres) atomicAnd(&amask[b >> 6], ~(1ull << (b & 63)));
    }
}
__global__ void __launch_bounds__(64) k_exact_norms(const float *__restrict__ dfa, const float *__restrict__ dfb, float *__restrict__ out, WMask which, Geo g) {
    const int b = blockIdx.x, lane = threadIdx.x;
    if (!which.test(b)) return;
    float fa, fd;
    exact_norms(dfa + b * g.es, dfb + b * g.es, g, lane, fa, fd);
    if (lane == 0) { out[2 * b] = fa; out[2 * b + 1] = fd; }
}
void launch_exact_norms(sfa_ctx *c, const Geo &g, const float *dfa, const float *dfb, const WMask &which, float *out) {
    hipLaunchKernelGGL(k_exact_norms, dim3(g.nb), dim3(64), 0, c->stream, dfa, dfb, out, which, g);
}
__global__ void k_set_mask(unsigned long long *amask, WMask v) { for (int i = 0; i < kMaskWords; i++) amask[i] = v.w[i]; }
static unsigned long long *unsure_of(sfa_ctx *c) { return c->d_last->unsure; }
void launch_outer_threshold(sfa_ctx *c, const Geo &g, const double *red, float thres, const float *dfa, const float *dfb) {
    const bool exact = dfa && thres > 0.0f;
    hipLaunchKernelGGL(k_outer_threshold, dim3(kMaskWords), dim3(64), 0, c->stream, red, c->d_last->last, c->d_amask, g.active, g.nb, (double)g.h * g.w, thres,
                       exact ? unsure_of(c) : (unsigned long long *)nullptr, break_band(g.w, g.h));
    if (exact) hipLaunchKernelGGL(k_exact_break, dim3(g.nb), dim3(64), 0, c->stream, dfa, dfb, c->d_last->last, c->d_amask, unsure_of(c), g, thres);
}
void launch_set_mask(sfa_ctx *c, const WMask &v) { hipLaunchKernelGGL(k_set_mask, dim3(1), dim3(1), 0, c->stream, c->d_amask, v); }

static double *partials_of(sfa_ctx *c) { return c->d_red + 2 * kMaxBatch; }
constexpr int kRedRows = 16;
static inline dim3 red_grid(const Geo &g, int z) { return dim3((g.w + BX - 1) / BX, std::min((g.h + BY - 1) / BY, kRedRows), z); }

void launch_update_inner(sfa_ctx *c, const Geo &g, float *uu, float *vv, const float *wx, const float *wy, const float *du, const float *dv,
                         const float *old_du, const float *old_dv, double *red, float *dfa, float *dfb) {
    dim3 grid = red_grid(g, g.nb);
    const int per_elem = grid.x * grid.y;
    hipLaunchKernelGGL(k_update_inner, grid, block2d(), 0, c->stream, uu, vv, wx, wy, du, dv, old_du, old_dv, partials_of(c), dfa, dfb, g);
    hipLaunchKernelGGL(k_reduce_partials, dim3(g.nb), dim3(256), 0, c->stream, partials_of(c), per_elem, red, g.active, g.amask);
}
void launch_update_inner_x(sfa_ctx *c, const Geo &g, float *uu, float *vv, const float *wx, const float *wy, const SorOperandOut &x, const float *old_du,
                           const float *old_dv, float *du_out, float *dv_out, double *red, float *dfa, float *dfb) {
    dim3 grid = red_grid(g, g.nb);
    const int per_elem = grid.x * grid.y;
    hipLaunchKernelGGL(k_update_inner_x, grid, block2d(), 0, c->stream, uu, vv, wx, wy, x.x, x.ent, x.RP, x.G, old_du, old_dv, du_out, dv_out, partials_of(c), dfa, dfb, g);
    hipLaunchKernelGGL(k_reduce_partials, dim3(g.nb), dim3(256), 0, c->stream, partials_of(c), per_elem, red, g.active, g.amask);
}
constexpr int kFuseReduceWindows = 4;
void launch_update_outer_x(sfa_ctx *c, const Geo &g, float *uu, float *vv, float *wx, float *wy, const SorOperandOut &x, double *red, float *dfa, float *dfb) {
    dim3 grid((g.w + 63) / 64, std::min((g.h + 15) / 16, kRedRows), g.nb);
    const int per_elem = grid.x * grid.y;
    unsigned *done = c->d_last->done;
    if (g.nb <= kFuseReduceWindows) {
        hipLaunchKernelGGL(k_update_outer_x<true>, grid, block2d(), 0, c->stream, uu, vv, wx, wy, x.x, x.ent, x.RP, x.G, partials_of(c), red, done, dfa, dfb, g);
        return;
    }
    hipLaunchKernelGGL(k_update_outer_x<false>, grid, block2d(), 0, c->stream, uu, vv, wx, wy, x.x, x.ent, x.RP, x.G, partials_of(c), red, done, dfa, dfb, g);
    hipLaunchKernelGGL(k_reduce_partials, dim3(g.nb), dim3(256), 0, c->stream, partials_of(c), per_elem, red, g.active, g.amask);
}
void launch_update_outer(sfa_ctx *c, const Geo &g, float *wx, float *wy, const float *uu, const float *vv, double *red, float *dfa, float *dfb) {
    dim3 grid = red_grid(g, g.nb);
    const int per_elem = grid.x * grid.y;
    hipLaunchKernelGGL(k_update_outer, grid, block2d(), 0, c->stream, wx, wy, uu, vv, partials_of(c), dfa, dfb, g);
    hipLaunchKernelGGL(k_reduce_partials, dim3(g.nb), dim3(256), 0, c->stream, partials_of(c), per_elem, red, g.active, g.amask);
}

__global__ void k_copy_planes(float *__restrict__ dst, const float *__restrict__ src, Geo g, int nplanes, long dst_es, long src_es) {
    const int b = blockIdx.z / nplanes, pl = blockIdx.z % nplanes;
    if (!elem_active(g, b)) return;
    const int x = blockIdx.x * BX + threadIdx.x, y = blockIdx.y * BY + threadIdx.y;
    if (x >= g.w || y >= g.h) return;
    const size_t o = pl * g.pl + (size_t)y * g.pitch + x;
    dst[b * dst_es + o] = src[b * src_es + o];
}
void launch_copy_planes(sfa_ctx *c, const Geo &g, float *dst, const float *src, int nplanes, long dst_es, long src_es) {
    hipLaunchKernelGGL(k_copy_planes, grid2d(g, nplanes), block2d(), 0, c->stream, dst, src, g, nplanes, dst_es, src_es);
}

__global__ void k_fill_planes(float *__restrict__ p, Geo g, int nplanes, float v) {
    const int b = blockIdx.z / nplanes, pl = blockIdx.z % nplanes;
    if (!elem_active(g, b)) return;
    const int x = blockIdx.x * BX + threadIdx.x, y = blockIdx.y * BY + threadIdx.y;
    if (x >= g.pitch || y >= g.h) return;
    p[b * g.es + pl * g.pl + (size_t)y * g.pitch + x] = v;
}
void launch_fill_planes(sfa_ctx *c, const Geo &g, float *p, int nplanes, float v) {
    dim3 grid((g.pitch + BX - 1) / BX, (g.h + BY - 1) / BY, g.nb * nplanes);
    hipLaunchKernelGGL(k_fill_planes, grid, block2d(), 0, c->stream, p, g, nplanes, v);
}
void launch_zero_planes(sfa_ctx *c, const Geo &g, float *p, int nplanes) { launch_fill_planes(c, g, p, nplanes, 0.0f); }

__global__ void k_scale_plane(float *__restrict__ p, Geo g, float s) {
    const int b = blockIdx.z;
    const int x = blockIdx.x * BX + threadIdx.x, y = blockIdx.y * BY + threadIdx.y;
    if (x >= g.w || y >= g.h) return;
    p[b * g.es + (size_t)y * g.pitch + x] *= s;
}
void launch_scale_plane(sfa_ctx *c, const Geo &g, float *p, float s) {
    hipLaunchKernelGGL(k_scale_plane, grid2d(g), block2d(), 0, c->stream, p, g, s);
}

struct Taps { float k[17]; int r; };

__global__ void k_gauss_h(float *__restrict__ dst, const float *__restrict__ src, Geo g, int nplanes, Taps t) {
    const int b = blockIdx.z / nplanes, pl = blockIdx.z % nplanes;
    const int x = blockIdx.x * BX + threadIdx.x, y = blockIdx.y * BY + threadIdx.y;
    if (x >= g.w || y >= g.h) return;
    const float *s = src + b * g.es + pl * g.pl + (size_t)y * g.pitch;
    float acc = t.k[t.r] * s[x];
    for (int j = 1; j <= t.r; j++) acc += t.k[t.r + j] * (s[clampi(x - j, 0, g.w - 1)] + s[clampi(x + j, 0, g.w - 1)]);
    dst[b * g.es + pl * g.pl + (size_t)y * g.pitch + x] = acc;
}
__global__ void k_gauss_v(float *__restrict__ dst, const float *__restrict__ src, Geo g, int nplanes, Taps t) {
    const int b = blockIdx.z / nplanes, pl = blockIdx.z % nplanes;
    const int x = blockIdx.x * BX + threadIdx.x, y = blockIdx.y * BY + threadIdx.y;
    if (x >= g.w || y >= g.h) return;
    const float *s = src + b * g.es + pl * g.pl;
    float acc = t.k[t.r] * s[(size_t)y * g.pitch + x];
    for (int j = 1; j <= t.r; j++)
        acc += t.k[t.r + j] * (s[(size_t)clampi(y - j, 0, g.h - 1) * g.pitch + x] + s[(size_t)clampi(y + j, 0, g.h - 1) * g.pitch + x]);
    dst[b * g.es + pl * g.pl + (size_t)y * g.pitch + x] = acc;
}
void launch_gauss_blur(sfa_ctx *c, const Geo &g, float *dst, float *tmp, const float *src, int nplanes, const float *taps, int radius) {
    Taps t;
    t.r = radius;
    for (int i = 0; i < 2 * radius + 1; i++) t.k[i] = taps[i];
    hipLaunchKernelGGL(k_gauss_h, grid2d(g, nplanes), block2d(), 0, c->stream, tmp, src, g, nplanes, t);
    hipLaunchKernelGGL(k_gauss_v, grid2d(g, nplanes), block2d(), 0, c->stream, dst, tmp, g, nplanes, t);
}

__global__ void k_resize(float *__restrict__ dst, int dw, int dh, int dpitch, long dpl, long des, const float *__restrict__ src, int sw, int sh, int spitch,
                         long spl, long ses, int nplanes, double scale_x, double scale_y, float post_scale) {
    const int b = blockIdx.z / nplanes, pl = blockIdx.z % nplanes;
    const int dx = blockIdx.x * BX + threadIdx.x, dy = blockIdx.y * BY + threadIdx.y;
    if (dx >= dw || dy >= dh) return;
    float fx = (float)((dx + 0.5) * scale_x - 0.5);
    int sx = (int)floorf(fx);
    fx -= sx;
    if (sx < 0) { fx = 0; sx = 0; }
    if (sx >= sw - 1) { fx = 0; sx = sw - 1; }
    float fy = (float)((dy + 0.5) * scale_y - 0.5);
    int sy = (int)floorf(fy);
    fy -= sy;
    if (sy < 0) { fy = 0; sy = 0; }
    if (sy >= sh - 1) { fy = 0; sy = sh - 1; }
    const int sx1 = sx + 1 < sw ? sx + 1 : sx, sy1 = sy + 1 < sh ? sy + 1 : sy;
    const float *s = src + b * ses + pl * spl;
    const float *r0 = s + (size_t)sy * spitch, *r1 = s + (size_t)sy1 * spitch;
    const float a0 = 1.f - fx, a1 = fx, b0 = 1.f - fy, b1 = fy;
    const float h0 = r0[sx] * a0 + r0[sx1] * a1;
    const float h1 = r1[sx] * a0 + r1[sx1] * a1;
    float v = h0 * b0 + h1 * b1;
    if (post_scale != 1.0f) v *= post_scale;
    dst[b * des + pl * dpl + (size_t)dy * dpitch + dx] = v;
}
void launch_resize_scaled(sfa_ctx *c, float *dst, int dw, int dh, int dpitch, long dpl, long des, const float *src, int sw, int sh, int spitch, long spl,
                          long ses, int nplanes, int nb, float post_scale, double scale_x, double scale_y) {
    dim3 grid((dw + BX - 1) / BX, (dh + BY - 1) / BY, nb * nplanes);
    hipLaunchKernelGGL(k_resize, grid, block2d(), 0, c->stream, dst, dw, dh, dpitch, dpl, des, src, sw, sh, spitch, spl, ses, nplanes, scale_x, scale_y, post_scale);
}
void launch_resize(sfa_ctx *c, float *dst, int dw, int dh, int dpitch, long dpl, long des, const float *src, int sw, int sh, int spitch, long spl, long ses,
                   int nplanes, int nb, float post_scale) {
    launch_resize_scaled(c, dst, dw, dh, dpitch, dpl, des, src, sw, sh, spitch, spl, ses, nplanes, nb, post_scale, (double)sw / dw, (double)sh / dh);
}

constexpr int kRfRows = 16;
__global__ void __launch_bounds__(BX * 4) k_resize_flow(float *__restrict__ dx_, float *__restrict__ dy_, int dw, int dh, int dpitch, long des, const float *__restrict__ sx_,
                                                         const float *__restrict__ sy_, int sw, int sh, int spitch, long ses, double scale_x, double scale_y, float post_x,
                                                         float post_y) {
    __shared__ int s_sy[kRfRows], s_sy1[kRfRows];
    __shared__ float s_fy[kRfRows];
    const int b = blockIdx.z;
    const int dx = blockIdx.x * BX + threadIdx.x, dy0 = blockIdx.y * kRfRows;
    if (threadIdx.y == 0 && threadIdx.x < kRfRows) {
        const int dy = dy0 + threadIdx.x;
        float fy = (float)((dy + 0.5) * scale_y - 0.5);
        int sy = (int)floorf(fy);
        fy -= sy;
        if (sy < 0) { fy = 0; sy = 0; }
        if (sy >= sh - 1) { fy = 0; sy = sh - 1; }
        s_sy[threadIdx.x] = sy; s_sy1[threadIdx.x] = sy + 1 < sh ? sy + 1 : sy; s_fy[threadIdx.x] = fy;
    }
    __syncthreads();
    if (dx >= dw) return;
    float fx = (float)((dx + 0.5) * scale_x - 0.5);
    int sx = (int)floorf(fx);
    fx -= sx;
    if (sx < 0) { fx = 0; sx = 0; }
    if (sx >= sw - 1) { fx = 0; sx = sw - 1; }
    const int sx1 = sx + 1 < sw ? sx + 1 : sx;
    const float a0 = 1.f - fx, a1 = fx;
    const float *px = sx_ + b * ses, *py = sy_ + b * ses;
#pragma unroll
    for (int k = 0; k < kRfRows / 4; k++) {
        const int ry = threadIdx.y + 4 * k, dy = dy0 + ry;
        if (dy >= dh) break;
        const size_t o0 = (size_t)s_sy[ry] * spitch, o1 = (size_t)s_sy1[ry] * spitch;
        const float fy = s_fy[ry], b0 = 1.f - fy, b1 = fy;
        const float x00 = px[o0 + sx], x01 = px[o0 + sx1], x10 = px[o1 + sx], x11 = px[o1 + sx1];
        const float y00 = py[o0 + sx], y01 = py[o0 + sx1], y10 = py[o1 + sx], y11 = py[o1 + sx1];
        float vx = (x00 * a0 + x01 * a1) * b0 + (x10 * a0 + x11 * a1) * b1;
        float vy = (y00 * a0 + y01 * a1) * b0 + (y10 * a0 + y11 * a1) * b1;
        if (post_x != 1.0f) vx *= post_x;
        if (post_y != 1.0f) vy *= post_y;
        const size_t o = b * des + (size_t)dy * dpitch + dx;
        dx_[o] = vx; dy_[o] = vy;
    }
}
void launch_resize_flow(sfa_ctx *c, float *dstx, float *dsty, int dw, int dh, int dpitch, long des, const float *srcx, const float *srcy, int sw, int sh, int spitch,
                        long ses, int nb, float post_x, float post_y) {
// ... 285 lines not shown
```

slowflow_amd/csrc/sfa_device.h:

```cpp
#pragma once
#include "sfa_internal.h"

#pragma clang fp contract(off)

namespace sfa {

#define BX 64
#define BY 4

static inline dim3 grid2d(const Geo &g, int zmul = 1) { return dim3((g.w + BX - 1) / BX, (g.h + BY - 1) / BY, g.nb * zmul); }
static inline dim3 block2d() { return dim3(BX, BY, 1); }

__device__ __forceinline__ bool elem_active(const WMask &active, const unsigned long long *amask, int b) {
    const unsigned long long m = amask ? (active.w[b >> 6] & amask[b >> 6]) : active.w[b >> 6];
    return (m >> (b & 63)) & 1ull;
}
__device__ __forceinline__ bool elem_active(const Geo &g, int b) { return elem_active(g.active, g.amask, b); }
__device__ __forceinline__ int clampi(int a, int lo, int hi) { return a < lo ? lo : (a > hi ? hi : a); }
__device__ __forceinline__ int floor_to_int_x86(float v) {
    const float f = floorf(v);
    return (f >= -2147483648.0f && f < 2147483648.0f) ? (int)f : (-2147483647 - 1);
}

#define C5_0 (1.0f / 12.0f)
#define C5_1 (-8.0f / 12.0f)
#define C5_2 (-0.0f)
#define C5_3 (8.0f / 12.0f)
#define C5_4 (-(1.0f / 12.0f))
#define C3_0 (-0.5f)
#define C3_1 (-0.0f)
#define C3_2 (0.5f)

__device__ __forceinline__ float tap5(float m2, float m1, float c, float p1, float p2) {
#if defined(SFA_X_NO_CENTRE_TAP)
    return C5_0 * m2 + C5_1 * m1 + C5_3 * p1 + C5_4 * p2;
#else
    return C5_0 * m2 + C5_1 * m1 + C5_2 * c + C5_3 * p1 + C5_4 * p2;
#endif
}

template <class F>
__device__ __forceinline__ float d5x(F f, int x, int y, int w) {
    return tap5(f(clampi(x - 2, 0, w - 1), y), f(clampi(x - 1, 0, w - 1), y), f(x, y), f(clampi(x + 1, 0, w - 1), y), f(clampi(x + 2, 0, w - 1), y));
}
template <class F>
__device__ __forceinline__ float d5y(F f, int x, int y, int h) {
    if (y == 0) return (C5_0 + C5_1 + C5_2) * f(x, 0) + C5_3 * f(x, 1) + C5_4 * f(x, 2);
    if (y == 1) return (C5_0 + C5_1) * f(x, 0) + C5_2 * f(x, 1) + C5_3 * f(x, 2) + C5_4 * f(x, 3);
    if (y == h - 2) return C5_0 * f(x, y - 2) + C5_1 * f(x, y - 1) + C5_2 * f(x, y) + (C5_3 + C5_4) * f(x, y + 1);
    if (y == h - 1) return C5_0 * f(x, y - 2) + C5_1 * f(x, y - 1) + (C5_2 + C5_3 + C5_4) * f(x, y);
    return tap5(f(x, y - 2), f(x, y - 1), f(x, y), f(x, y + 1), f(x, y + 2));
}
template <class F>
__device__ __forceinline__ float d3x(F f, int x, int y, int w) {
    return C3_0 * f(clampi(x - 1, 0, w - 1), y) + C3_1 * f(x, y) + C3_2 * f(clampi(x + 1, 0, w - 1), y);
}
template <class F>
__device__ __forceinline__ float d3y(F f, int x, int y, int h) {
    if (y == 0) return (C3_0 + C3_1) * f(x, 0) + C3_2 * f(x, 1);
    if (y == h - 1) return C3_0 * f(x, y - 1) + (C3_1 + C3_2) * f(x, y);
    return C3_0 * f(x, y - 1) + C3_1 * f(x, y) + C3_2 * f(x, y + 1);
}

__device__ __forceinline__ float sqrt_rn(float x) { return __builtin_sqrtf(x); }

struct PlaneAcc {
    const float *p; int pitch;
    __device__ __forceinline__ float operator()(int x, int y) const { return p[(size_t)y * pitch + x]; }
};

template <class T2>
__device__ __forceinline__ void bilinear2(const T2 *__restrict__ p, int w, int h, double x, double y, double &ru, double &rv) {
    const int y0 = (int)y, x0 = (int)x;
    int y1 = y0, x1 = x0;
    double wx = 0, wy = 0;
    if (x0 + 1 < w) { wx = x - x0; x1++; }
    if (y0 + 1 < h) { wy = y - y0; y1++; }
    const T2 a = p[(size_t)y0 * w + x0], b = p[(size_t)y0 * w + x1];
    const T2 c = p[(size_t)y1 * w + x0], d = p[(size_t)y1 * w + x1];
    ru = (1 - wy) * (1 - wx) * (double)a.x + (1 - wy) * wx * (double)b.x + wy * (1 - wx) * (double)c.x + wy * wx * (double)d.x;
    rv = (1 - wy) * (1 - wx) * (double)a.y + (1 - wy) * wx * (double)b.y + wy * (1 - wx) * (double)c.y + wy * wx * (double)d.y;
}

}
```

slowflow_amd/csrc/sfa_internal.h:

```cpp
#pragma once
#include <hip/hip_runtime.h>

#include <cstdarg>
#include <cstdio>
#include <string>
#include <vector>

#include "../../include/slowflow_amd.h"
#include "dev_view.h"

#pragma clang fp contract(off)

namespace sfa {

constexpr int kMaskWords = 2;
constexpr int kMaxBatch = 64 * kMaskWords;
struct WMask {
    unsigned long long w[kMaskWords];
    __host__ __device__ bool test(int b) const { return (w[b >> 6] >> (b & 63)) & 1ull; }
    __host__ __device__ void clear(int b) { w[b >> 6] &= ~(1ull << (b & 63)); }
    __host__ __device__ void set(int b) { w[b >> 6] |= 1ull << (b & 63); }
    __host__ __device__ bool any() const { unsigned long long o = 0; for (int i = 0; i < kMaskWords; i++) o |= w[i]; return o != 0; }
    __host__ __device__ bool operator==(const WMask &o) const { bool e = true; for (int i = 0; i < kMaskWords; i++) e = e && w[i] == o.w[i]; return e; }
    __host__ __device__ bool operator!=(const WMask &o) const { return !(*this == o); }
    __host__ __device__ WMask operator&(const WMask &o) const { WMask r; for (int i = 0; i < kMaskWords; i++) r.w[i] = w[i] & o.w[i]; return r; }
    __host__ __device__ WMask andnot(const WMask &o) const { WMask r; for (int i = 0; i < kMaskWords; i++) r.w[i] = w[i] & ~o.w[i]; return r; }
    int count() const { int n = 0; for (int i = 0; i < kMaskWords; i++) n += __builtin_popcountll(w[i]); return n; }
    static WMask none() { WMask r; for (int i = 0; i < kMaskWords; i++) r.w[i] = 0; return r; }
    static WMask first(int nb) {
        WMask r;
        for (int i = 0; i < kMaskWords; i++) r.w[i] = nb >= 64 * (i + 1) ? ~0ull : nb <= 64 * i ? 0ull : (1ull << (nb - 64 * i)) - 1;
        return r;
    }
    static WMask one(int b) { WMask r = none(); r.w[b >> 6] = 1ull << (b & 63); return r; }
};
constexpr int kMaxTerms = 4 * SFA_MAX_REF;
struct LastBlock {
    double last[2 * kMaxBatch];
    unsigned done[kMaxBatch];
    unsigned long long unsure[kMaskWords];
    float exact[2 * kMaxBatch];
};
__host__ __device__ inline double break_band(int w, int h) {
    const double bound = (double)((w + 3) / 4) * (double)h * (1.0 / 16777216.0);
    return bound > 1e-3 ? bound : 1e-3;
}

constexpr int kMaskLag = 2, kMaskRing = 4;
static_assert(kMaskLag < kMaskRing, "a ring slot is rewritten kMaskRing iterations after it was read kMaskLag iterations late");

struct DevBlock { void *p; size_t bytes; };

}

struct sfa_ctx {
    int device = 0;
    hipStream_t stream = nullptr;
    std::string err;
    double *d_red = nullptr;
    double *h_red = nullptr;
    unsigned long long *d_amask = nullptr;
    sfa::LastBlock *d_last = nullptr;
    sfa::WMask *h_amask = nullptr;
    hipEvent_t ev_mask[sfa::kMaskRing] = {};
    unsigned *d_err = nullptr;
    bool profile = false;
    std::vector<hipEvent_t> ev;
    size_t ev_used = 0;
    double sor_bytes = 0;
    std::vector<hipEvent_t> ev2;
    size_t ev2_used = 0;
    double asm_pixel_terms = 0;
    char sor_kernel[160] = {0};
    void *rb_tmp = nullptr;
    size_t rb_tmp_bytes = 0;
    void *q_tmp = nullptr;
    size_t q_tmp_bytes = 0;
    hipEvent_t t0 = nullptr, t1 = nullptr;
    hipEvent_t ev_wait = nullptr, ev_signal = nullptr;
    bool verbose_changes = false;
    int cu_count = 256;
};

namespace sfa {

constexpr int kRedDoubles = 1 << 20;

int set_error(sfa_ctx *ctx, int code, const char *fmt, ...);
extern thread_local std::string g_thread_err;

struct Switches {
    enum Id {
        SOR_CHAIN, SOR_BAND, SOR_F, SOR_CH, SOR_LEAD, CHAIN_LDS, RB_TILE, WARP_ALLJ, NO_WARP_SMOOTH, ASSEMBLE_GENERIC, EXACT_DIV, ASM_XCD, NO_DIRECT_OPERANDS,
        NO_UV_ALIAS, DEBUG_ACTIVE, UNFUSED, SHARE_SOR, PYRAMID_UNFUSED, CUT_DISCHARGE, CUT_INNER, CUT_SUPER, CUT_TAIL_INNER, CUT_PER, CUT_TAIL_PER, CUT_TAIL_SUPER,
        CUT_DEBUG, CUT_NO_TAIL, CUT_TAIL, NO_EXACT_BREAK, PAIR_UNFUSED, N
    };
    bool given[N] = {};
    int value[N] = {};
};
#ifdef SFA_RELEASE
#define SFA_FULL(...)
#else
#define SFA_FULL(...) __VA_ARGS__
#endif
#ifdef SFA_RELEASE
constexpr bool sw_given(Switches::Id) { return false; }
constexpr int sw_int(Switches::Id, int dflt) { return dflt; }
#else
extern Switches g_switches;
inline bool sw_given(Switches::Id i) { return g_switches.given[i]; }
inline int sw_int(Switches::Id i, int dflt) { return g_switches.given[i] ? g_switches.value[i] : dflt; }
#endif

#define SFA_HIP(ctx, call)                                                                         \
    do {                                                                                           \
        hipError_t _e = (call);                                                                    \
        if (_e != hipSuccess)                                                                      \
            return sfa::set_error((ctx), SFA_ERR_HIP, "%s failed: %s (%s:%d)", #call, hipGetErrorString(_e), __FILE__, __LINE__); \
    } while (0)

#define SFA_TRY(expr)            \
    do {                         \
        int _rc = (expr);        \
        if (_rc != SFA_OK) return _rc; \
    } while (0)

#define CHECK_ARGS_FN(fn, cond, msg) do { if (!(cond)) return sfa::set_error(ctx, SFA_ERR_ARG, "%s: %s", fn, msg); } while (0)
#define CHECK_ARGS(cond, msg) CHECK_ARGS_FN(__func__, cond, msg)
#define REFUSE(...) return sfa::set_error(ctx, SFA_ERR_ARG, __VA_ARGS__)

inline int round_up(int a, int m) { return (a + m - 1) / m * m; }
inline int host_stride(int w) { return ((w + 3) / 4) * 4; }
#ifndef SFA_PITCH_ODD
#define SFA_PITCH_ODD 0
#endif
inline int dev_pitch(int w) { const int p = round_up(w, 64); return (SFA_PITCH_ODD && ((p / 64) & 1) == 0) ? p + 64 : p; }

struct DevMem {
    void *p = nullptr;
    size_t bytes = 0;
    DevMem() = default;
    DevMem(const DevMem &) = delete;
    DevMem &operator=(const DevMem &) = delete;
    ~DevMem() { release(); }
    int alloc(sfa_ctx *ctx, size_t n);
    void release();
    float *f() const { return static_cast<float *>(p); }
};

int upload_plane(sfa_ctx *ctx, float *dev, int pitch, const float *host, int stride, int w, int h);
int download_plane(sfa_ctx *ctx, float *host, int stride, const float *dev, int pitch, int w, int h);

int jet_source_check(sfa_ctx *ctx, const char *fn, const sfa_jet_source *src, int w, int h, bool *identity);
int jet_resample_flows(sfa_ctx *ctx, const sfa_jet_source &src, size_t np, const float *const *u, const float *const *v, int w, int h, float *stage, double2 *out,
                       hipEvent_t before, hipEvent_t after);
int jet_decode_occlusions(sfa_ctx *ctx, const sfa_jet_source &src, size_t np, const unsigned char *const *occ, int w, int h, unsigned char *stage, unsigned char *out);
int launch_jet_resample(sfa_ctx *ctx, const sfa_jet_source &src, size_t np, const float *su, const float *sv, int w, int h, double2 *out);
int launch_jet_occ_decode(sfa_ctx *ctx, const sfa_jet_source &src, size_t np, const unsigned char *stage, int w, int h, unsigned char *out);

void launch_interleave(sfa_ctx *ctx, const float *u, const float *v, float2 *out, size_t n);
int accumulate_device(sfa_ctx *ctx, int n, int FF, int w, int h, int gw, int gh, int skip, bool identity, const void *fwd, const void *bwd,
                      const unsigned char *masks, double epsilon, int discard, int all_steps, double *acc_u, double *acc_v, int *tracked);
struct AdaptTab {
    int off[32], offm1[32];
    float skip;
    int up;
};
struct EnergyArgs {
    double acc_jc, acc_cv, acc_bc, acc_gc, acc_occ, acc_temporal_occ;
    float thr, fb_thr;
    int penalty;
    double eps_sq;
    float weight;
};
struct EnergyPlan { AdaptTab tab; EnergyArgs a; int rJ, J, w, h, gw, gh, incr, start, r, NN; size_t lds; };
int energy_plan(sfa_ctx *ctx, const sfa_energy_params *p, int r_Jets, int Jets, int w, int h, EnergyPlan *out);
void energy_records_device(sfa_ctx *ctx, size_t nf, int w, int h, const float *frames, float *der, void *rec);
struct EnergyWork { double *U, *V; unsigned long long *occ; float *jc, *oc; double *ep; };
int energies_device(sfa_ctx *ctx, const EnergyPlan &pl, int n, const double *acc_u, const double *acc_v, const int *tracked, const void *rec, bool identity,
                    const void *fwd, const void *bwd, const EnergyWork &wk, double *energy, unsigned long long *occ_out, size_t out_seg, double *adapted_u,
                    double *adapted_v, size_t adapted_seg);
int energies_adapted_device(sfa_ctx *ctx, const EnergyPlan &pl, int n, const int *tracked, const EnergyWork &wk, double *adapted_u, double *adapted_v, size_t adapted_seg);
struct FuseWork {
    const double *U, *V, *energy; const unsigned long long *occ; const float *weight;
    unsigned char *nl, *lab; double *theta, *P, *M; unsigned char *xcur, *xbest;
    int *slot; double *fu, *fv; unsigned char *out_occ; double *seg_energy, *seg_bound; int *seg_iters;
};
int fuse_device(sfa_ctx *ctx, const sfa_fuse_params *p, int n, int K, int Jets, int w, int h, int gw, int gh, const FuseWork &f, hipEvent_t *ev);

struct Geo { int w, h, pitch; long pl; long es; int nb; WMask active; const unsigned long long *amask; };

struct PenaltyDev { int id; float eps, trunc; };
inline PenaltyDev pen(const sfa_penalty &p) { return PenaltyDev{p.id, p.eps, p.trunc}; }

struct WarpJob { long src_off, dst_off, mask_off; int factor; };
struct WarpJobs { WarpJob job[4 * SFA_MAX_REF]; int n; };
void launch_warp_jobs(sfa_ctx *c, const Geo &g, const WarpJobs &J, float *base, const float *wx, const float *wy);
bool launch_warp_smooth(sfa_ctx *c, const Geo &g, const WarpJobs &J, float *base, const float *wx, const float *wy, int method, float *sh, float *sv,
                        const float *dpsis, float alpha, PenaltyDev reg);
void launch_warp(sfa_ctx *c, const Geo &g, float *dst3, float *mask, const float *src3, const float *wx, const float *wy, int factor,
                 long src_es );
void launch_deriv_stack(sfa_ctx *c, const Geo &g, float *out24, const float *I1, const float *I2, long es1, long es2);
void launch_convolve(sfa_ctx *c, const Geo &g, float *dst, const float *src, int order, int horiz, int nplanes);
void launch_dpsis(sfa_ctx *c, const Geo &g, float *dst, const float *im3, long im_es, float coef, const float avg[3], const float stdv[3], int hbit);
void launch_smoothness(sfa_ctx *c, const Geo &g, int method, float *sh, float *sv, const float *uu, const float *vv, const float *dpsis,
                       float alpha, PenaltyDev reg);
void launch_sub_laplacian(sfa_ctx *c, const Geo &g, float *dst, const float *src, const float *wh, const float *wv);
void launch_mask_weight(sfa_ctx *c, const Geo &g, float *masks, const float *occ, float data_norm, int ref, int one_direction);
void launch_fill(sfa_ctx *c, float *p, size_t n, float v);
void launch_division_chain(sfa_ctx *c, const float *a, const float *b, float *q_chain, float *q_exact, unsigned char *admitted, size_t n);
void launch_fill_planes(sfa_ctx *c, const Geo &g, float *p, int nplanes, float v);
void launch_zero_planes(sfa_ctx *c, const Geo &g, float *p, int nplanes);
void launch_outer_threshold(sfa_ctx *c, const Geo &g, const double *red, float thres, const float *dfa = nullptr, const float *dfb = nullptr);
void launch_set_mask(sfa_ctx *c, const WMask &v);

struct SorOperandOut {
    float4 *sa = nullptr, *sb = nullptr; unsigned long long *x = nullptr; unsigned *flags = nullptr;
    long ent = 0; int RP = 0, G = 0, ntasks = 0, nb = 0;
};
struct Term {
    long stack_off; long mask_off; float hd, hg, s; int is_ref;
    long i1_off, i2_off; int backward;
};
struct AssembleArgs {
    Term t[kMaxTerms];
    int n;
    int dt_norm;
    PenaltyDev color, grad;
    const float *chw; long chw_pl; long chw_es; int chw_pitch; int chw_stride0; int lstride;
    int accumulate;
    int do_laplacian;
    float data_norm; int one_direction;
    SorOperandOut op;
    int zero_duv;
    int chain_ok = 0;
};
void launch_assemble(sfa_ctx *c, const Geo &g, const AssembleArgs &a, const float *base , float *a11, float *a12,
                     float *a22, float *b1, float *b2, const float *du, const float *dv, const float *uu, const float *vv, const float *sh, const float *sv);

int launch_assemble_images(sfa_ctx *c, const Geo &g, const AssembleArgs &a, const float *base, float *a11, float *a12, float *a22, float *b1, float *b2,
                            const float *du, const float *dv, const float *uu, const float *vv, const float *sh, const float *sv, const float *occ);

void launch_smoothness_2f(sfa_ctx *c, const Geo &g, float *sh, float *sv, const float *uu, const float *vv, const float *dpsis, float half_alpha);
void launch_data_2f(sfa_ctx *c, const Geo &g, const float *D, const float *mask, const float *du, const float *dv, float *a11, float *a12, float *a22, float *b1,
                    float *b2, const float *wx, const float *wy, const float *sh, const float *sv, float hd, float hg);
void launch_data_2f_fused(sfa_ctx *c, const Geo &g, const float *I1, const float *I2, const float *mask, const float *du, const float *dv, float *a11, float *a12,
                          float *a22, float *b1, float *b2, const float *wx, const float *wy, const float *sh, const float *sv, float hd, float hg);

struct OccSlot {
    long s1_off, s2_off;
    long r1_off, r2_off;
    long mask_off;
    float rho, omega;
    int label;
};
struct OccArgs { OccSlot slot[2 * SFA_MAX_REF]; int nslots; float hd, hg, penalty; PenaltyDev color, grad; };
void launch_occ_costs(sfa_ctx *c, const Geo &g, const OccArgs &a, const float *base, float *d0, float *d1, long d_es );
constexpr int kCutWorkPlanes = 13;
int run_grid_cut(sfa_ctx *c, const Geo &g, float *occ, long occ_es, const float *d0, const float *d1, float *work, float alpha);

void launch_update_inner(sfa_ctx *c, const Geo &g, float *uu, float *vv, const float *wx, const float *wy, const float *du, const float *dv,
                         const float *old_du, const float *old_dv, double *red , float *dfa = nullptr, float *dfb = nullptr);
void launch_update_inner_x(sfa_ctx *c, const Geo &g, float *uu, float *vv, const float *wx, const float *wy, const SorOperandOut &x, const float *old_du,
                           const float *old_dv, float *du_out, float *dv_out, double *red, float *dfa = nullptr, float *dfb = nullptr);
void launch_exact_norms(sfa_ctx *c, const Geo &g, const float *dfa, const float *dfb, const WMask &which, float *out);
void launch_update_outer_x(sfa_ctx *c, const Geo &g, float *uu, float *vv, float *wx, float *wy, const SorOperandOut &x, double *red, float *dfa = nullptr,
                           float *dfb = nullptr);
void launch_update_outer(sfa_ctx *c, const Geo &g, float *wx, float *wy, const float *uu, const float *vv, double *red, float *dfa = nullptr, float *dfb = nullptr);
void launch_copy_planes(sfa_ctx *c, const Geo &g, float *dst, const float *src, int nplanes, long dst_es, long src_es);
void launch_scale_plane(sfa_ctx *c, const Geo &g, float *p, float s);

void launch_gauss_blur(sfa_ctx *c, const Geo &g, float *dst, float *tmp, const float *src, int nplanes, const float *taps, int radius);
void launch_resize(sfa_ctx *c, float *dst, int dw, int dh, int dpitch, long dpl, long des, const float *src, int sw, int sh, int spitch, long spl, long ses,
                   int nplanes, int nb, float post_scale);
void launch_resize_flow(sfa_ctx *c, float *dstx, float *dsty, int dw, int dh, int dpitch, long des, const float *srcx, const float *srcy, int sw, int sh, int spitch,
                        long ses, int nb, float post_x, float post_y);
void launch_resize_scaled(sfa_ctx *c, float *dst, int dw, int dh, int dpitch, long dpl, long des, const float *src, int sw, int sh, int spitch, long spl,
                          long ses, int nplanes, int nb, float post_scale, double scale_x, double scale_y);
bool launch_pyr_down(sfa_ctx *c, float *dst, int dw, int dh, int dpitch, long dpl, long des, const float *src, int sw, int sh, int spitch, long spl, long ses,
                     int nplanes, int nb, const float *taps, int radius);
void launch_presmooth(sfa_ctx *c, const Geo &g, float *dst, float *tmp, const float *src, int nplanes, float sigma);
void launch_normalize_sums(sfa_ctx *c, const Geo &g, const float *frames3, double *red );
void launch_normalize_apply(sfa_ctx *c, const Geo &g, float *frames3, const double avg[3], const double stdv[3]);
__attribute__((visibility("hidden"))) int cv_gauss_taps(float sigma, float *k);

struct PackSrc { const void *p; int dtype; long long sw, sf, sc, sr, sx; };
void launch_pack_frames(sfa_ctx *c, float *dst, long dst_es, long pl, int pitch, int w, int h, int nwin, int F, const PackSrc &s);
void launch_pack_flow(sfa_ctx *c, float *dst, long dst_es, long pl, int pitch, int w, int h, int nwin, const float *src, const long long st[4]);
void launch_unpack_planes(sfa_ctx *c, const float *wx, const float *wy, const float *occ, long src_es, int pitch, int w, int h, int nwin, float *flow,
                          const long long st[4], float *occ_dst, const long long ost[3]);

struct MosaicSrc { const void *p; int dtype; long long sf, sr, sx; int W, H, x0, y0; };
struct MosaicDst { float *p; long long sf, sc, sr, sx; int w, h; };
void launch_demosaic(sfa_ctx *c, const MosaicSrc &src, const MosaicDst &dst, int n, int method, int red_x, int red_y);
void launch_raw_weights(sfa_ctx *c, float *chw, long es, long pl, int cp, int stride, int w, int h, int nwin, int red_x, int red_y, float weight);

struct SorWorkspace {
    sfa_ctx *ctx = nullptr;
    int w = 0, h = 0, K = 0, nb = 0;
    int NB = 0, NG = 0, RP = 0, ND = 0, G = 0, NS = 0, NCH = 0, ntasks = 0, F = 0, CHK = 0;
    int nwords = 0;
    long ent = 0;
    int band = 0, Wp = 0, EP = 0;
    int chain = 0;
    long edge_job = 0;
    DevMem sa, sb, x, flags, order, edge;
    int configure(sfa_ctx *ctx, int w, int h, int K, int nb);
};
int sor_operand_target(sfa_ctx *c, SorWorkspace &ws, const Geo &g, int K, SorOperandOut *out);
int sor_run_prepared(sfa_ctx *c, SorWorkspace &ws, const Geo &g, float *du, float *dv, int K, float omega);
int sor_rb_run(sfa_ctx *c, const Geo &g, float *du, float *dv, float *a11, float *a12, float *a22, const float *b1, const float *b2, const float *sh,
               const float *sv, int K, float omega);
int sor_run(sfa_ctx *c, SorWorkspace &ws, const Geo &g, float *du, float *dv, float *a11, float *a12, float *a22, const float *b1, const float *b2,
            const float *sh, const float *sv, int K, float omega, bool inv_out);

__attribute__((visibility("hidden"))) int check_view(sfa_ctx *ctx, const char *fn, const View &v, long long min_inner = 1);
__attribute__((visibility("hidden"))) int check_disjoint(sfa_ctx *ctx, const char *fn, std::initializer_list<View> views, const char *why = nullptr);
int check_frames_source(sfa_ctx *ctx, const char *fn, const void *frames_dev, const sfa_dev_layout *l, long long win_stride, int nwin, int F, int w, int h);
int check_device_pointer(sfa_ctx *ctx, const char *fn, const char *arg, const void *p, long long last, size_t elem);
int check_download_destination(sfa_ctx *ctx, const char *fn, int n, int w, int h, float *flow_dev, const long long strides[4], float *occ_dev,
                               const long long occ_strides[3]);
int check_batch_range(sfa_ctx *ctx, const char *fn, const char *what, int b0, int n, int nb);
__attribute__((visibility("hidden"))) int check_mosaic_method(sfa_ctx *ctx, const char *fn, int method, int red_x, int red_y);

}

struct sfa_pair_job {
    enum { WX, WY, UU, VV, DU, DV, SH, SV, A11, A12, A22, B1, B2, MASK, DPS, IM1, IM2 = IM1 + 3, WIM2 = IM2 + 3, NPL = WIM2 + 3 };
    sfa_ctx *ctx = nullptr;
    int w = 0, h = 0, n = 0, pitch = 0;
    long pl = 0, es = 0;
    sfa_params_2frame p;
    bool stored_stack = false;
    sfa::DevMem mem;
    sfa::DevMem stack;
    sfa::SorWorkspace ws;
    float *plane(int b, int i) const { return mem.f() + b * es + (long)i * pl; }
    sfa::Geo geo() const { return sfa::Geo{w, h, pitch, pl, es, n, sfa::WMask::first(n), nullptr}; }
};

struct sfa_sequence {
    sfa_ctx *ctx = nullptr;
    int w = 0, h = 0, n = 0, pitch = 0;
    long pl = 0;
    sfa::DevMem mem;
    sfa::DevMem sums;
    void *mos_stage = nullptr;
    size_t mos_stage_bytes = 0;
    hipEvent_t ev_mos = nullptr;
    sfa::DevMem mos_dev;
    sfa::DevMem rescale_tmp;
    float *frame(int f) const { return mem.f() + (long)f * 3 * pl; }
    sfa::Geo geo() const { return sfa::Geo{w, h, pitch, pl, 0, 1, sfa::WMask::first(1), nullptr}; }
};
```

Baseline: 264,400.

## Skip dead occlusion loads, norm reductions and operand writes when unused

When occlusion reasoning is off, the occlusion plane is constant, so mask weights are computed once on the host and a specialized assemble kernel skips the per-pixel occlusion load. Outer flow-update norms and the reduction are skipped unless thresholds, verbose output or the final change report need them. The zero-initial-guess operand write becomes a constant store. A persistent occlusion plane is filled once at job creation instead of every level. Derivative taps with zero coefficients now go through an fma helper, which may change rounding and adds branching surface.

```diff
diff --git a/slowflow_amd/csrc/api.hip b/slowflow_amd/csrc/api.hip
--- a/slowflow_amd/csrc/api.hip
+++ b/slowflow_amd/csrc/api.hip
@@ -18,7 +18,7 @@
     "SFA_SOR_CHAIN", "SFA_SOR_BAND", "SFA_SOR_F", "SFA_SOR_CH", "SFA_SOR_LEAD", "SFA_CHAIN_LDS", "SFA_RB_TILE", "SFA_WARP_ALLJ", "SFA_NO_WARP_SMOOTH",
     "SFA_ASSEMBLE_GENERIC", "SFA_EXACT_DIV", "SFA_ASM_XCD", "SFA_NO_DIRECT_OPERANDS", "SFA_NO_UV_ALIAS", "SFA_DEBUG_ACTIVE", "SFA_UNFUSED", "SFA_SHARE_SOR",
     "SFA_PYRAMID_UNFUSED", "SFA_CUT_DISCHARGE", "SFA_CUT_INNER", "SFA_CUT_SUPER", "SFA_CUT_TAIL_INNER", "SFA_CUT_PER", "SFA_CUT_TAIL_PER", "SFA_CUT_TAIL_SUPER",
-    "SFA_CUT_DEBUG", "SFA_CUT_NO_TAIL", "SFA_CUT_TAIL", "SFA_NO_EXACT_BREAK", "SFA_PAIR_UNFUSED"};
+    "SFA_CUT_DEBUG", "SFA_CUT_NO_TAIL", "SFA_CUT_TAIL", "SFA_NO_EXACT_BREAK", "SFA_PAIR_UNFUSED", "SFA_KEEP_DEAD_WORK"};
 static int set_switch(const char *name, const char *value) {
     for (int i = 0; i < Switches::N; i++)
         if (!strcmp(name, kSwitchNames[i])) {
diff --git a/slowflow_amd/csrc/job.hip b/slowflow_amd/csrc/job.hip
--- a/slowflow_amd/csrc/job.hip
+++ b/slowflow_amd/csrc/job.hip
@@ -18,7 +18,8 @@
     long off_masks = 0, off_warp = 0, off_stacks = 0, off_tmp = 0;
     float *base = nullptr;
     float *pbase = nullptr;
-    float *plane(int i) const { return i < 2 ? pbase + (long)i * pl : base + (long)(i - 2) * pl; }
+    float *obase = nullptr;
+    float *plane(int i) const { return i == P_OCC && obase ? obase : i < 2 ? pbase + (long)i * pl : base + (long)(i - 2) * pl; }
     float *mask(int s) const { return base + off_masks + (long)s * pl; }
     float *stack(int s, int toref) const { return base + off_stacks + ((long)s * 2 + toref) * 24 * pl; }
     float *warp(int s, int sp1) const { return base + off_warp + (long)(s + sp1) * 3 * pl; }
@@ -30,8 +31,8 @@
     static long transient_floats(int pitch, int h, int ref, bool fused) {
         return (long)pitch * h * ((P_COUNT - 2) + 2 * ref + (2L * ref + 1) * 3 + (fused ? 0 : 2L * ref * 2 * 24));
     }
-    void layout(float *transient, float *persistent, int w_, int h_, int lstride_, int ref_, int nb_, long es_, bool fused_) {
-        base = transient; pbase = persistent; w = w_; h = h_; pitch = dev_pitch(w_); lstride = lstride_; ref = ref_; F = 2 * ref_ + 1; nb = nb_; es = es_; fused = fused_;
+    void layout(float *transient, float *persistent, float *occlusion, int w_, int h_, int lstride_, int ref_, int nb_, long es_, bool fused_) {
+        base = transient; pbase = persistent; obase = occlusion; w = w_; h = h_; pitch = dev_pitch(w_); lstride = lstride_; ref = ref_; F = 2 * ref_ + 1; nb = nb_; es = es_; fused = fused_;
         pl = (long)pitch * h;
         off_masks = (long)(P_COUNT - 2) * pl;
         off_warp = off_masks + 2L * ref * pl;
@@ -86,6 +87,8 @@
     return run_grid_cut(c, g, L.plane(P_OCC), L.es, d0, d1, work, p.occlusion_alpha);
 }
 
+static float occ_fill(const sfa_params &p) { return (p.one_direction || p.occlusion_reasoning) ? -1.0f : 0.0f; }
+
 
 static Term data_term(const Level &L, const sfa_params &p, int slot, int is_ref, float weight, float s) {
     const float *i1 = pair_image(L, slot, 0), *i2 = pair_image(L, slot, 1);
@@ -93,7 +96,7 @@
     return Term{L.off_stacks + ((long)slot * 2 + is_ref) * 24 * L.pl, L.off_masks + (long)slot * L.pl, weight * (p.delta / 3.0f), weight * (p.gamma / 3.0f), s, is_ref,
                 i1 - L.base, i2 - L.base, slot < L.ref};
 }
-static int data_terms(sfa_ctx *c, const Level &L, const sfa_params &p, const ChannelWeights &cw, AssembleArgs &aa, bool need_toref[2 * SFA_MAX_REF]) {
+static int data_terms(sfa_ctx *c, const Level &L, const sfa_params &p, const ChannelWeights &cw, bool const_occ, AssembleArgs &aa, bool need_toref[2 * SFA_MAX_REF]) {
     const int ref = L.ref;
     memset(&aa, 0, sizeof aa);
     for (int s = 0; s < ref; s++) {
@@ -112,6 +115,8 @@
     aa.color = pen(p.robust_color); aa.grad = pen(p.robust_grad);
     aa.chw = cw.dev; aa.chw_pl = cw.pl; aa.chw_es = cw.es; aa.chw_pitch = cw.pitch; aa.chw_stride0 = cw.stride0; aa.lstride = L.lstride;
     aa.accumulate = 0; aa.do_laplacian = 1;
+    aa.const_occ = const_occ ? 1 : 0;
+    if (const_occ) mask_weights(occ_fill(p), aa.data_norm, aa.fwd, aa.bwd);
     return SFA_OK;
 }
 
@@ -121,6 +126,7 @@
     bool direct;
     bool uv_alias;
     bool thres_in, thres_out;
+    bool lean, const_occ;
     float *wx, *wy, *uu, *vv, *du, *dv, *odu, *odv, *sh, *sv, *a11, *a12, *a22, *b1, *b2, *occ, *dpsis, *UU, *VV;
     float *dfa, *dfb, *ifa, *ifb;
     LevelPlan(const sfa_ctx *c, const Level &L, const sfa_params &p) {
@@ -129,6 +135,7 @@
         direct = L.fused && !red_black && !sw_given(Switches::NO_DIRECT_OPERANDS);
         uv_alias = direct && p.niter_inner == 1 && !sw_given(Switches::NO_UV_ALIAS) && !verbose;
         thres_in = p.thres_inner > 0; thres_out = p.thres_outer > 0;
+        lean = !sw_given(Switches::KEEP_DEAD_WORK); const_occ = lean && !p.occlusion_reasoning;
         wx = L.plane(P_WX); wy = L.plane(P_WY); uu = L.plane(P_UU); vv = L.plane(P_VV); du = L.plane(P_DU); dv = L.plane(P_DV);
         odu = L.plane(P_ODU); odv = L.plane(P_ODV); sh = L.plane(P_SH); sv = L.plane(P_SV); a11 = L.plane(P_A11); a12 = L.plane(P_A12);
         a22 = L.plane(P_A22); b1 = L.plane(P_B1); b2 = L.plane(P_B2); occ = L.plane(P_OCC); dpsis = L.plane(P_DPSIS);
@@ -136,6 +143,7 @@
         dfa = thres_out && !sw_given(Switches::NO_EXACT_BREAK) ? a11 : nullptr; dfb = dfa ? a12 : nullptr;
         ifa = thres_in && !sw_given(Switches::NO_EXACT_BREAK) ? a11 : nullptr; ifb = ifa ? a12 : nullptr;
     }
+    bool want_norms(bool last_iter, const float *change) const { return !lean || verbose || thres_out || (last_iter && change); }
 };
 
 struct OuterBreak {
@@ -181,11 +189,11 @@
     return sor_run(c, sorws, gi, P.du, P.dv, P.a11, P.a12, P.a22, P.b1, P.b2, P.sh, P.sv, p.niter_solver, p.sor_omega, false);
 }
 
-static bool update_flow(sfa_ctx *c, const sfa_params &p, const LevelPlan &P, const SorOperandOut &x, const Geo &gi, int inner, bool first_zero) {
+static bool update_flow(sfa_ctx *c, const sfa_params &p, const LevelPlan &P, const SorOperandOut &x, const Geo &gi, int inner, bool first_zero, bool norms) {
     const bool last = inner + 1 == p.niter_inner;
     float *const ia = last ? nullptr : P.ifa, *const ib = last ? nullptr : P.ifb;
     if (P.direct && last && !P.verbose) {
-        launch_update_outer_x(c, gi, P.uv_alias ? nullptr : P.uu, P.uv_alias ? nullptr : P.vv, P.wx, P.wy, x, c->d_red, P.dfa, P.dfb);
+        launch_update_outer_x(c, gi, P.uv_alias ? nullptr : P.uu, P.uv_alias ? nullptr : P.vv, P.wx, P.wy, x, norms ? c->d_red : nullptr, P.dfa, P.dfb);
         return true;
     }
     if (P.direct)
@@ -218,7 +226,8 @@
     return SFA_OK;
 }
 
-static int inner_iterations(sfa_ctx *c, const Level &L, const sfa_params &p, const LevelPlan &P, AssembleArgs &aa, SorWorkspace &sorws, const Geo &g, bool smoothed) {
+static int inner_iterations(sfa_ctx *c, const Level &L, const sfa_params &p, const LevelPlan &P, AssembleArgs &aa, SorWorkspace &sorws, const Geo &g, bool smoothed,
+                            bool norms) {
     if (!P.direct) launch_zero_planes(c, g, P.du, 2);
     WMask in_active = g.active, outer_done = WMask::none();
     for (int inner = 0; inner < p.niter_inner; inner++) {
@@ -226,7 +235,7 @@
         gi.active = in_active;
         const bool first_zero = P.direct && inner == 0;
         SFA_TRY(assemble_and_solve(c, L, p, P, aa, sorws, gi, first_zero, smoothed && inner == 0));
-        if (update_flow(c, p, P, aa.op, gi, inner, first_zero)) outer_done = in_active;
+        if (update_flow(c, p, P, aa.op, gi, inner, first_zero, norms)) outer_done = in_active;
         if (P.verbose) print_changes(c, L, "\tinner it", inner, in_active);
         if (P.thres_in && inner + 1 < p.niter_inner) {
             SFA_TRY(inner_break(c, L, p, P, gi, in_active));
@@ -243,12 +252,12 @@
 static int run_level(sfa_ctx *c, const Level &L, const sfa_params &p, const ChannelWeights &cw, SorWorkspace &sorws, DevMem &cut_scratch, float *change, float *occ_log) {
     AssembleArgs aa;
     bool need_toref[2 * SFA_MAX_REF] = {false};
-    SFA_TRY(data_terms(c, L, p, cw, aa, need_toref));
     const LevelPlan P(c, L, p);
+    SFA_TRY(data_terms(c, L, p, cw, P.const_occ, aa, need_toref));
     const OuterBreak brk{c, P.thres_out};
     const WMask all = WMask::first(L.nb);
     Geo g = L.geo(all);
-    launch_fill_planes(c, g, P.occ, 1, (p.one_direction || p.occlusion_reasoning) ? -1.0f : 0.0f);
+    if (!P.const_occ) launch_fill_planes(c, g, P.occ, 1, occ_fill(p));
     launch_dpsis(c, g, P.dpsis, L.frame(L.ref), L.es, 5.0f, p.norm_avg, p.norm_std, p.hbit);
     if (!P.uv_alias) launch_copy_planes(c, g, P.uu, P.wx, 2, L.es, L.es);
     g.amask = c->d_amask;
@@ -270,10 +279,11 @@
             g.active = active;
             if (outer > 0) smoothed = get_derivatives(c, L, p, g, need_toref, P.uv_alias);
             if (!L.fused) launch_mask_weight(c, g, L.mask(0), P.occ, aa.data_norm, L.ref, p.one_direction);
-            SFA_TRY(inner_iterations(c, L, p, P, aa, sorws, g, smoothed));
+            const bool last_iter = (alter == p.niter_alter - 1 && outer == p.niter_outer - 1);
+            const bool norms = P.want_norms(last_iter, change);
+            SFA_TRY(inner_iterations(c, L, p, P, aa, sorws, g, smoothed, norms));
             if (P.verbose) print_changes(c, L, "outer it", outer, active);
-            const bool last_iter = (alter == p.niter_alter - 1 && outer == p.niter_outer - 1);
-            if (P.thres_out || last_iter) launch_outer_threshold(c, g, c->d_red, P.thres_out ? p.thres_outer : 0.0f, P.dfa, P.dfb);
+            if (P.thres_out || (last_iter && norms)) launch_outer_threshold(c, g, c->d_red, P.thres_out ? p.thres_outer : 0.0f, P.dfa, P.dfb);
             SFA_TRY(brk.publish(outer));
         }
     }
@@ -312,6 +322,7 @@
     long es = 0;
     std::vector<long> level_off;
     long trans_off = 0;
+    long occ_off = 0;
     bool share_sor = false;
     DevMem arena;
     DevMem init_flow;
@@ -326,7 +337,7 @@
     bool fused = true;
     Level level(int l) const {
         Level Lv;
-        Lv.layout(arena.f() + trans_off, arena.f() + level_off[l], ws[l], hs[l], l == 0 ? host_stride0 : host_stride(ws[l]), ref, nb, es, fused);
+        Lv.layout(arena.f() + trans_off, arena.f() + level_off[l], p.occlusion_reasoning ? nullptr : arena.f() + occ_off, ws[l], hs[l], l == 0 ? host_stride0 : host_stride(ws[l]), ref, nb, es, fused);
         return Lv;
     }
     WMask presmoothed = WMask::none();
@@ -439,11 +450,17 @@
     }
     j->trans_off = off;
     off += Level::transient_floats(dev_pitch(j->ws[0]), j->hs[0], j->ref, j->fused);
+    j->occ_off = off;
+    if (!p->occlusion_reasoning) off += (long)dev_pitch(j->ws[0]) * j->hs[0];
     j->es = off;
     j->share_sor = (double)w * h >= 2.0e6 || sw_given(Switches::SHARE_SOR);
     j->host_stride0 = host_stride(w);
     SFA_TRY(j->arena.alloc(ctx, (size_t)batch * j->es * sizeof(float)));
     SFA_HIP(ctx, hipMemsetAsync(j->arena.p, 0, (size_t)batch * j->es * sizeof(float), ctx->stream));
+    if (!p->occlusion_reasoning && occ_fill(*p) != 0.0f) {
+        const Level L0 = j->level(0);
+        launch_fill_planes(ctx, L0.geo(), L0.plane(P_OCC), 1, occ_fill(*p));
+    }
     SFA_TRY(j->init_flow.alloc(ctx, (size_t)batch * 2 * dev_pitch(w) * h * sizeof(float)));
     SFA_HIP(ctx, hipMemsetAsync(j->init_flow.p, 0, (size_t)batch * 2 * dev_pitch(w) * h * sizeof(float), ctx->stream));
     j->change.assign(2 * batch, 0.f);
diff --git a/slowflow_amd/csrc/kernels.hip b/slowflow_amd/csrc/kernels.hip
--- a/slowflow_amd/csrc/kernels.hip
+++ b/slowflow_amd/csrc/kernels.hip
@@ -723,12 +723,6 @@
                        b2, wx, wy, sh, sv, g, hd, hg);
 }
 
-__device__ __forceinline__ void mask_weights(float oc, float data_norm, float &fwd, float &bwd) {
-    float factor = (oc == 0.0f) ? 1.0f : 0.0f;
-    factor = (1 + factor) * data_norm;
-    bwd = __fdiv_rn((oc >= 0.0f) ? 1.0f : 0.0f, factor);
-    fwd = __fdiv_rn((oc <= 0.0f) ? 1.0f : 0.0f, factor);
-}
 __global__ void k_mask_weight(float *__restrict__ masks, const float *__restrict__ occ, Geo g, float data_norm, int ref, int one_direction) {
     const int b = blockIdx.z;
     if (!elem_active(g, b)) return;
@@ -1332,7 +1326,7 @@
     }
     return p;
 }
-template <class K>
+template <class K, bool XZ>
 __device__ __forceinline__ void asm_epilogue_pixel(const AssembleArgs &a, const Geo &g, Acc &A, float u, float v, int x0, int y0, int tx, int yl, int x, int y) {
     const float *const lds = asm_lds<K>();
     const int gy0 = y0 + DT_H - 1;
@@ -1350,9 +1344,9 @@
     const OperandTile<K> T;
     T.A[yl][tx] = make_float4(q.i11, q.i12, q.i22, vt);
     T.B[yl][tx] = make_float4(A.b1, A.b2, hp, y < g.h - 1 ? vp : 0.0f);
-    T.X[yl][tx] = make_float2(u, v);
-}
-template <class K>
+    if (!XZ) T.X[yl][tx] = make_float2(u, v);
+}
+template <class K, bool XZ>
 __device__ __forceinline__ void asm_store_operand_tile(const SorOperandOut &op, const Geo &g, int b, int c0, int r0) {
     const OperandTile<K> T;
     for (int item = threadIdx.x; item < (DT_X + K::TY - 1) * K::TY; item += K::NT) {
@@ -1362,14 +1356,14 @@
         if (r >= g.h || c >= g.w) continue;
         const size_t e = diag_entry(b, op.ent, op.RP, op.G, c, r);
         if (SFA_X_AI & 64) continue;
-        const float2 xv = T.X[rl][cl];
         op.sa[e] = T.A[rl][cl];
         op.sb[e] = T.B[rl][cl];
-        op.x[e] = f2u(xv.x, xv.y);
-    }
-}
-
-template <int TY, int NT, int MINB, bool ZUV, int FAST, bool XT>
+        if (XZ) op.x[e] = 0ull;
+        else { const float2 xv = T.X[rl][cl]; op.x[e] = f2u(xv.x, xv.y); }
+    }
+}
+
+template <int TY, int NT, int MINB, bool ZUV, int FAST, bool XT, bool CW>
 __global__ void __launch_bounds__(NT, MINB) k_assemble_images(AssembleArgs a, const float *__restrict__ base, float *__restrict__ a11, float *__restrict__ a12,
                                                               float *__restrict__ a22, float *__restrict__ b1, float *__restrict__ b2,
                                                               const float *__restrict__ du, const float *__restrict__ dv, const float *__restrict__ uu,
@@ -1408,7 +1402,7 @@
         const size_t o = (size_t)y * g.pitch + x;
         if (!ZUV) { u[k] = du[eb + o]; v[k] = dv[eb + o]; }
         if (!FAST && a.chw) channel_weights(a, b, x, y, wk[k]);
-        if (!(SFA_X_AI & 128)) oc[k] = occ[eb + o];
+        if (!CW && !(SFA_X_AI & 128)) oc[k] = occ[eb + o];
     }
     const bool need_g = a.do_laplacian || a.op.sa;
     auto stage_epilogue_operands = [&]() {
@@ -1441,7 +1435,8 @@
         asm volatile("s_waitcnt vmcnt(0)" ::: "memory");
 #pragma unroll
         for (int k = 0; k < NP; k++) {
-            asm volatile("" : "+v"(mk[k]), "+v"(oc[k]));
+            if (CW) asm volatile("" : "+v"(mk[k]));
+            else asm volatile("" : "+v"(mk[k]), "+v"(oc[k]));
             if (!FAST) asm volatile("" : "+v"(wk[k][0]), "+v"(wk[k][1]), "+v"(wk[k][2]));
             if (!ZUV) asm volatile("" : "+v"(u[k]), "+v"(v[k]));
         }
@@ -1450,7 +1445,10 @@
         AT_MARK(4);
         if (t == 0) {
 #pragma unroll
-            for (int k = 0; k < NP; k++) mask_weights(oc[k], a.data_norm, fwd[k], bwd[k]);
+            for (int k = 0; k < NP; k++) {
+                if (CW) { fwd[k] = a.fwd; bwd[k] = a.bwd; }
+                else mask_weights(oc[k], a.data_norm, fwd[k], bwd[k]);
+            }
         }
         if (tile_in) asm_convert<K, true>(base + eb + T.i1_off, base + eb + T.i2_off, g, x0, y0);
         else asm_convert<K, false>(base + eb + T.i1_off, base + eb + T.i2_off, g, x0, y0);
@@ -1495,7 +1493,7 @@
     for (int k = 0; k < NP; k++) {
         if (!ok[k]) continue;
         const int yl = ty + NR * k, y = y0 + DT_H + yl;
-        asm_epilogue_pixel<K>(a, g, A[k], u[k], v[k], x0, y0, tx, yl, x, y);
+        asm_epilogue_pixel<K, ZUV && CW>(a, g, A[k], u[k], v[k], x0, y0, tx, yl, x, y);
         if (!a.op.sa) {
             const size_t o = eb + (size_t)y * g.pitch + x;
             a11[o] = A[k].a11; a12[o] = A[k].a12; a22[o] = A[k].a22; b1[o] = A[k].b1; b2[o] = A[k].b2;
@@ -1505,18 +1503,20 @@
     AT_MARK(10);
     __syncthreads();
     AT_MARK(11);
-    asm_store_operand_tile<K>(a.op, g, b, x0 + DT_H, y0 + DT_H);
+    asm_store_operand_tile<K, ZUV && CW>(a.op, g, b, x0 + DT_H, y0 + DT_H);
 #ifdef SFA_ASM_TIMING
     AT_MARK(12);
     if ((threadIdx.x & 63) == 0 && (bx + 3 * by + 7 * b) % 61 == 0)
         for (int i = 0; i < 14; i++) atomicAdd(&g_asm_timing[i], at_acc[i]);
 #endif
 }
-using AsmKernel = decltype(&k_assemble_images<kAsmTY, kAsmNT, kAsmMinWaves, true, 1, true>);
+using AsmKernel = decltype(&k_assemble_images<kAsmTY, kAsmNT, kAsmMinWaves, true, 1, true, false>);
 template <bool ZUV, int FAST>
 static AsmKernel asm_kernel(bool xcd) {
-    return xcd ? k_assemble_images<kAsmTY, kAsmNT, kAsmMinWaves, ZUV, FAST, true> : k_assemble_images<kAsmTY, kAsmNT, kAsmMinWaves, ZUV, FAST, false>;
-}
+    return xcd ? k_assemble_images<kAsmTY, kAsmNT, kAsmMinWaves, ZUV, FAST, true, false> : k_assemble_images<kAsmTY, kAsmNT, kAsmMinWaves, ZUV, FAST, false, false>;
+}
+template <bool ZUV, int FAST>
+static AsmKernel asm_kernel_cw() { return k_assemble_images<kAsmTY, kAsmNT, kAsmMinWaves, ZUV, FAST, true, true>; }
 int launch_assemble_images(sfa_ctx *c, const Geo &g, const AssembleArgs &a_in, const float *base, float *a11, float *a12, float *a22, float *b1, float *b2,
                            const float *du, const float *dv, const float *uu, const float *vv, const float *sh, const float *sv, const float *occ) {
     AssembleArgs a = a_in;
@@ -1539,7 +1539,10 @@
     const bool xcd = xcd_env && ntiles >= 64 && ntiles < (1l << 30);
     const XcdTiles xt{(int)grid_.x, (int)grid_.y, (int)((ntiles + 7) / 8)};
     const dim3 grid1_(8u * (unsigned)xt.chunk, 1, 1);
-    const AsmKernel kern = a.zero_duv ? (fast == 1 ? asm_kernel<true, 1>(xcd) : fast == 2 ? asm_kernel<true, 2>(xcd) : asm_kernel<true, 0>(xcd))
+    const bool cw = a.const_occ && fast != 0 && xcd;
+    const AsmKernel kern = cw ? (a.zero_duv ? (fast == 1 ? asm_kernel_cw<true, 1>() : asm_kernel_cw<true, 2>())
+                                            : (fast == 1 ? asm_kernel_cw<false, 1>() : asm_kernel_cw<false, 2>()))
+                         : a.zero_duv ? (fast == 1 ? asm_kernel<true, 1>(xcd) : fast == 2 ? asm_kernel<true, 2>(xcd) : asm_kernel<true, 0>(xcd))
                                       : (fast == 1 ? asm_kernel<false, 1>(xcd) : fast == 2 ? asm_kernel<false, 2>(xcd) : asm_kernel<false, 0>(xcd));
     hipLaunchKernelGGL(kern, xcd ? grid1_ : grid_, dim3(kAsmNT), 0, c->stream, a, base, a11, a12, a22, b1, b2, du, dv, uu, vv, sh, sv, occ, g, xt);
     if (prof) {
@@ -1617,7 +1620,7 @@
         partial[2 * blk] = sa; partial[2 * blk + 1] = sb;
     }
 }
-template <bool FUSE>
+template <bool FUSE, bool NORMS>
 __global__ void __launch_bounds__(BX *BY) k_update_outer_x(float *__restrict__ uu, float *__restrict__ vv, float *__restrict__ wx, float *__restrict__ wy,
                                                             const unsigned long long *__restrict__ xs, long ent, int RP, int G, double *__restrict__ partial,
                                                             double *__restrict__ out, unsigned *__restrict__ done, float *__restrict__ dfa, float *__restrict__ dfb, Geo g) {
@@ -1648,10 +1651,12 @@
                     const float d = __uint_as_float((unsigned)(xv & 0xffffffffu)), e = __uint_as_float((unsigned)(xv >> 32));
                     const float ox = wx[o], oy = wy[o];
                     const float u = ox + d, v = oy + e;
-                    sa += (double)fabsf(u - ox);
-                    sb += (double)fabsf(v - oy);
+                    if (NORMS) {
+                        sa += (double)fabsf(u - ox);
+                        sb += (double)fabsf(v - oy);
+                    }
                     if (uu) { uu[o] = u; vv[o] = v; }
-                    if (dfa) { dfa[o] = fabsf(u - ox); dfb[o] = fabsf(v - oy); }
+                    if (NORMS && dfa) { dfa[o] = fabsf(u - ox); dfb[o] = fabsf(v - oy); }
 #if defined(SFA_UPD_NT) && SFA_UPD_NT
                     __builtin_nontemporal_store(u, wx + o); __builtin_nontemporal_store(v, wy + o);
 #else
@@ -1660,6 +1665,7 @@
                 }
         }
     }
+    if (!NORMS) return;
     block_sum2(sa, sb);
     if (!FUSE) {
         if (tid == 0) {
@@ -1832,11 +1838,16 @@
     dim3 grid((g.w + 63) / 64, std::min((g.h + 15) / 16, kRedRows), g.nb);
     const int per_elem = grid.x * grid.y;
     unsigned *done = c->d_last->done;
+    if (!red) {
+        hipLaunchKernelGGL((k_update_outer_x<false, false>), grid, block2d(), 0, c->stream, uu, vv, wx, wy, x.x, x.ent, x.RP, x.G, partials_of(c), red, done,
+                           (float *)nullptr, (float *)nullptr, g);
+        return;
+    }
     if (g.nb <= kFuseReduceWindows) {
-        hipLaunchKernelGGL(k_update_outer_x<true>, grid, block2d(), 0, c->stream, uu, vv, wx, wy, x.x, x.ent, x.RP, x.G, partials_of(c), red, done, dfa, dfb, g);
+        hipLaunchKernelGGL((k_update_outer_x<true, true>), grid, block2d(), 0, c->stream, uu, vv, wx, wy, x.x, x.ent, x.RP, x.G, partials_of(c), red, done, dfa, dfb, g);
         return;
     }
-    hipLaunchKernelGGL(k_update_outer_x<false>, grid, block2d(), 0, c->stream, uu, vv, wx, wy, x.x, x.ent, x.RP, x.G, partials_of(c), red, done, dfa, dfb, g);
+    hipLaunchKernelGGL((k_update_outer_x<false, true>), grid, block2d(), 0, c->stream, uu, vv, wx, wy, x.x, x.ent, x.RP, x.G, partials_of(c), red, done, dfa, dfb, g);
     hipLaunchKernelGGL(k_reduce_partials, dim3(g.nb), dim3(256), 0, c->stream, partials_of(c), per_elem, red, g.active, g.amask);
 }
 void launch_update_outer(sfa_ctx *c, const Geo &g, float *wx, float *wy, const float *uu, const float *vv, double *red, float *dfa, float *dfb) {
diff --git a/slowflow_amd/csrc/sfa_device.h b/slowflow_amd/csrc/sfa_device.h
--- a/slowflow_amd/csrc/sfa_device.h
+++ b/slowflow_amd/csrc/sfa_device.h
@@ -31,12 +31,10 @@
 #define C3_1 (-0.0f)
 #define C3_2 (0.5f)
 
+__device__ __forceinline__ float add_zero_tap(float s, float z, float c) { return __builtin_fmaf(z, c, s); }
+
 __device__ __forceinline__ float tap5(float m2, float m1, float c, float p1, float p2) {
-#if defined(SFA_X_NO_CENTRE_TAP)
-    return C5_0 * m2 + C5_1 * m1 + C5_3 * p1 + C5_4 * p2;
-#else
-    return C5_0 * m2 + C5_1 * m1 + C5_2 * c + C5_3 * p1 + C5_4 * p2;
-#endif
+    return add_zero_tap(C5_0 * m2 + C5_1 * m1, C5_2, c) + C5_3 * p1 + C5_4 * p2;
 }
 
 template <class F>
@@ -46,20 +44,20 @@
 template <class F>
 __device__ __forceinline__ float d5y(F f, int x, int y, int h) {
     if (y == 0) return (C5_0 + C5_1 + C5_2) * f(x, 0) + C5_3 * f(x, 1) + C5_4 * f(x, 2);
-    if (y == 1) return (C5_0 + C5_1) * f(x, 0) + C5_2 * f(x, 1) + C5_3 * f(x, 2) + C5_4 * f(x, 3);
-    if (y == h - 2) return C5_0 * f(x, y - 2) + C5_1 * f(x, y - 1) + C5_2 * f(x, y) + (C5_3 + C5_4) * f(x, y + 1);
+    if (y == 1) return add_zero_tap((C5_0 + C5_1) * f(x, 0), C5_2, f(x, 1)) + C5_3 * f(x, 2) + C5_4 * f(x, 3);
+    if (y == h - 2) return add_zero_tap(C5_0 * f(x, y - 2) + C5_1 * f(x, y - 1), C5_2, f(x, y)) + (C5_3 + C5_4) * f(x, y + 1);
     if (y == h - 1) return C5_0 * f(x, y - 2) + C5_1 * f(x, y - 1) + (C5_2 + C5_3 + C5_4) * f(x, y);
     return tap5(f(x, y - 2), f(x, y - 1), f(x, y), f(x, y + 1), f(x, y + 2));
 }
 template <class F>
 __device__ __forceinline__ float d3x(F f, int x, int y, int w) {
-    return C3_0 * f(clampi(x - 1, 0, w - 1), y) + C3_1 * f(x, y) + C3_2 * f(clampi(x + 1, 0, w - 1), y);
+    return add_zero_tap(C3_0 * f(clampi(x - 1, 0, w - 1), y), C3_1, f(x, y)) + C3_2 * f(clampi(x + 1, 0, w - 1), y);
 }
 template <class F>
 __device__ __forceinline__ float d3y(F f, int x, int y, int h) {
     if (y == 0) return (C3_0 + C3_1) * f(x, 0) + C3_2 * f(x, 1);
     if (y == h - 1) return C3_0 * f(x, y - 1) + (C3_1 + C3_2) * f(x, y);
-    return C3_0 * f(x, y - 1) + C3_1 * f(x, y) + C3_2 * f(x, y + 1);
+    return add_zero_tap(C3_0 * f(x, y - 1), C3_1, f(x, y)) + C3_2 * f(x, y + 1);
 }
 
 __device__ __forceinline__ float sqrt_rn(float x) { return __builtin_sqrtf(x); }
diff --git a/slowflow_amd/csrc/sfa_internal.h b/slowflow_amd/csrc/sfa_internal.h
--- a/slowflow_amd/csrc/sfa_internal.h
+++ b/slowflow_amd/csrc/sfa_internal.h
@@ -93,7 +93,7 @@
     enum Id {
         SOR_CHAIN, SOR_BAND, SOR_F, SOR_CH, SOR_LEAD, CHAIN_LDS, RB_TILE, WARP_ALLJ, NO_WARP_SMOOTH, ASSEMBLE_GENERIC, EXACT_DIV, ASM_XCD, NO_DIRECT_OPERANDS,
         NO_UV_ALIAS, DEBUG_ACTIVE, UNFUSED, SHARE_SOR, PYRAMID_UNFUSED, CUT_DISCHARGE, CUT_INNER, CUT_SUPER, CUT_TAIL_INNER, CUT_PER, CUT_TAIL_PER, CUT_TAIL_SUPER,
-        CUT_DEBUG, CUT_NO_TAIL, CUT_TAIL, NO_EXACT_BREAK, PAIR_UNFUSED, N
+        CUT_DEBUG, CUT_NO_TAIL, CUT_TAIL, NO_EXACT_BREAK, PAIR_UNFUSED, KEEP_DEAD_WORK, N
     };
     bool given[N] = {};
     int value[N] = {};
@@ -192,6 +192,18 @@
 
 struct PenaltyDev { int id; float eps, trunc; };
 inline PenaltyDev pen(const sfa_penalty &p) { return PenaltyDev{p.id, p.eps, p.trunc}; }
+
+__host__ __device__ __forceinline__ void mask_weights(float oc, float data_norm, float &fwd, float &bwd) {
+    float factor = (oc == 0.0f) ? 1.0f : 0.0f;
+    factor = (1 + factor) * data_norm;
+#ifdef __HIP_DEVICE_COMPILE__
+    bwd = __fdiv_rn((oc >= 0.0f) ? 1.0f : 0.0f, factor);
+    fwd = __fdiv_rn((oc <= 0.0f) ? 1.0f : 0.0f, factor);
+#else
+    bwd = ((oc >= 0.0f) ? 1.0f : 0.0f) / factor;
+    fwd = ((oc <= 0.0f) ? 1.0f : 0.0f) / factor;
+#endif
+}
 
 struct WarpJob { long src_off, dst_off, mask_off; int factor; };
 struct WarpJobs { WarpJob job[4 * SFA_MAX_REF]; int n; };
@@ -231,6 +243,7 @@
     int accumulate;
     int do_laplacian;
     float data_norm; int one_direction;
+    int const_occ; float fwd, bwd;
     SorOperandOut op;
     int zero_duv;
     int chain_ok = 0;
```

Measured after the change: 266,800, median of 6. Within noise of the previous version (+0.9%).
